# EmaMule/2D-to-3D-Style-Transfer

Measured on AMD Instinct MI355X. Metric: style-transfer iters/sec (512x512, 8 views, cow_mesh), higher is better.
Workload: dtype f32; 1 GPU; BASELINE.json configs[1]: cow_mesh + Style_1, 512x512, 8 views/GPU/iter, texture-only optimisation, white backgrounds (second_approach loop body); texture=512x512, targets_hoisted=content renders + content features + style Grams, parallelism=views sharded dp1, RCCL all-reduce of the texture gradient

## Files before the change

2d-to-3d-style-transfer_amd/csrc/need.hip:

```cpp
#include "common.h"

namespace {

typedef unsigned u32x4 __attribute__((ext_vector_type(4)));

__device__ __forceinline__ void need_segment(const uint8_t *__restrict__ mask, int S, int i, uint8_t *__restrict__ seg) {
    const int segs = S >> 6;
    const int sx = i % segs, y = (i / segs) % S, n = i / (segs * S);
    const uint8_t *m = mask + (size_t)n * S * S;
    unsigned any = 0;
    for (int dy = -1; dy <= 1; ++dy) {
        const int yy = y + dy;
        if (yy < 0 || yy >= S) continue;
        const uint8_t *row = m + (size_t)yy * S + 64 * sx;
        const u32x4 *q = reinterpret_cast<const u32x4 *>(row);
#pragma unroll
        for (int k = 0; k < 4; ++k) {
            const u32x4 v = q[k];
            any |= v[0] | v[1] | v[2] | v[3];
        }
        if (sx > 0) any |= row[-1];
        if (sx + 1 < segs) any |= row[64];
    }
    seg[i] = any ? 1 : 0;
}

__global__ __launch_bounds__(256) void need_segments_kernel(const uint8_t *__restrict__ mask, int S, int total,
                                                            uint8_t *__restrict__ seg) {
    const int i = blockIdx.x * 256 + threadIdx.x;
    if (i < total) need_segment(mask, S, i, seg);
}

struct NeedGeo {
    int tiles_x, tiles_y, rows, cols;
};

__device__ __forceinline__ unsigned seg_block_any(const uint8_t *__restrict__ seg, int S, int n, int ya, int yb, int sa, int sb) {
    const int segs = S >> 6;
    unsigned any = 0;
    for (int y = ya; y <= yb; ++y) {
        const uint8_t *row = seg + ((size_t)n * S + y) * segs;
#pragma unroll 4
        for (int s = sa; s <= sb; ++s) any |= row[s];
    }
    return any;
}

__global__ __launch_bounds__(64) void need_flags_kernel(const uint8_t *__restrict__ seg, int N, int S, NeedGeo g1, NeedGeo g2,
                                                        int total1, int total2, uint8_t *__restrict__ flags) {
    const int i = blockIdx.x * 64 + threadIdx.x;
    if (i >= total1 + total2) return;
    const bool second = i >= total1;
    const NeedGeo g = second ? g2 : g1;
    const int t = second ? i - total1 : i;
    const int per_img = g.tiles_x * g.tiles_y;
    const int n = t / per_img, r = t - n * per_img;
    const int ty = r / g.tiles_x, tx = r - ty * g.tiles_x;
    int ta = ty, tb = ty, ua = tx, ub = tx;
    if (second) {
        const int y0 = 2 * ty * g2.rows, y1 = y0 + 2 * g2.rows - 1;
        const int x0 = 2 * tx * g2.cols, x1 = x0 + 2 * g2.cols - 1;
        ta = max(0, (y0 - 1) / g1.rows); tb = min(g1.tiles_y - 1, (y1 + 1) / g1.rows);
        ua = max(0, (x0 - 1) / g1.cols); ub = min(g1.tiles_x - 1, (x1 + 1) / g1.cols);
    }
    flags[i] = seg_block_any(seg, S, n, ta * g1.rows, tb * g1.rows + g1.rows - 1, (ua * g1.cols) >> 6,
                             (ub * g1.cols + g1.cols - 1) >> 6) ? 1 : 0;
}

__global__ __launch_bounds__(1024) void need_lists_kernel(const uint8_t *__restrict__ flags, int total1, int total2,
                                                          int *__restrict__ list1, int *__restrict__ list2,
                                                          int *__restrict__ counts) {
    __shared__ int scan[1024];
    const int level = blockIdx.x, tid = threadIdx.x;
    const uint8_t *__restrict__ f = level == 0 ? flags : flags + total1;
    int *__restrict__ list = level == 0 ? list1 : list2;
    const int total = level == 0 ? total1 : total2;
    const int per = (total + 1023) / 1024;
    const int lo = min(total, tid * per), hi = min(total, lo + per);
    int cnt = 0;
    for (int t = lo; t < hi; ++t) cnt += f[t];
    scan[tid] = cnt;
    __syncthreads();
    for (int d = 1; d < 1024; d <<= 1) {
        const int v = tid >= d ? scan[tid - d] : 0;
        __syncthreads();
        scan[tid] += v;
        __syncthreads();
    }
    int o = scan[tid] - cnt;
    for (int t = lo; t < hi; ++t)
        if (f[t]) list[o++] = t;
    if (tid == 1023) counts[level] = scan[1023];
}

constexpr int kLists = ST3D_NEED_MAX_LISTS;
constexpr int kListShift[kLists] = {0, 1, 1, 2, 2, 2};
constexpr int kListUnpools[kLists] = {1, 0, 1, 0, 0, 0};

struct BlockLevels {
    int nlists;
    int first;
    int bw[kLists];
    int trows[kLists], tcols[kLists];
    int unpools[kLists];
    int N;
    int total[kLists + 1];
    int *list[kLists];
    int gram_runs;
    int *gram_list, *gram_count;
};

typedef unsigned long long u64;

__device__ __forceinline__ int row_words(int bw) { return (bw + 63) >> 6; }
__device__ __forceinline__ u64 row_tail_mask(int bw, int j) {
    const int left = bw - 64 * j;
    return left >= 64 ? ~0ull : (1ull << left) - 1ull;
}

__global__ __launch_bounds__(256) void need_front_kernel(const uint8_t *__restrict__ mask, int S, int seg_total, int seg_wgs,
                                                         uint8_t *__restrict__ seg, int b0_words, u64 *__restrict__ b0) {
    if ((int)blockIdx.x < seg_wgs) {
        const int i = blockIdx.x * 256 + threadIdx.x;
        if (i < seg_total) need_segment(mask, S, i, seg);
        return;
    }
    const int word = (blockIdx.x - seg_wgs) * 4 + (threadIdx.x >> 6), lane = threadIdx.x & 63;
    if (word >= b0_words) return;
    const int bw = S >> 2, W = row_words(bw);
    const int j = word % W, by = (word / W) % bw, n = word / (W * bw);
    const int bx = 64 * j + lane;
    unsigned any = 0;
    if (bx < bw) {
        const uint8_t *m = mask + (size_t)n * S * S + 4 * bx;
        const int left = bx > 0 ? -1 : 0, right = bx + 1 < bw ? 4 : 3;
#pragma unroll
        for (int r = -1; r <= 4; ++r) {
            const uint8_t *row = m + (size_t)min(max(4 * by + r, 0), S - 1) * S;
            any |= *reinterpret_cast<const unsigned *>(row) | row[left] | row[right];
        }
    }
    const u64 bits = __ballot(any != 0);
    if (lane == 0) b0[word] = bits;
}

__global__ __launch_bounds__(256) void kept_front_kernel(const uint8_t *__restrict__ cover, int S, int k0_words, u64 *__restrict__ k0) {
    const int word = blockIdx.x * 4 + (threadIdx.x >> 6), lane = threadIdx.x & 63;
    if (word >= k0_words) return;
    const int bw = S >> 2, W = row_words(bw);
    const int j = word % W, by = (word / W) % bw, n = word / (W * bw);
    const int bx = 64 * j + lane;
    unsigned any = 0;
    if (bx < bw) {
        const uint8_t *m = cover + (size_t)n * S * S + 4 * bx;
        const int l2 = bx > 0 ? -2 : 0, l1 = bx > 0 ? -1 : 0, r1 = bx + 1 < bw ? 4 : 3, r2 = bx + 1 < bw ? 5 : 3;
#pragma unroll
        for (int r = -2; r <= 5; ++r) {
            const uint8_t *row = m + (size_t)min(max(4 * by + r, 0), S - 1) * S;
            any |= *reinterpret_cast<const unsigned *>(row) | row[l2] | row[l1] | row[r1] | row[r2];
        }
    }
    const u64 bits = __ballot(any != 0);
    if (lane == 0) k0[word] = bits;
}

__device__ __forceinline__ u64 even_bits(u64 x) {
    x &= 0x5555555555555555ull;
    x = (x | (x >> 1)) & 0x3333333333333333ull;
    x = (x | (x >> 2)) & 0x0f0f0f0f0f0f0f0full;
    x = (x | (x >> 4)) & 0x00ff00ff00ff00ffull;
    x = (x | (x >> 8)) & 0x0000ffff0000ffffull;
    x = (x | (x >> 16)) & 0x00000000ffffffffull;
    return x;
}

template <int ROWS>
__device__ __forceinline__ u64 rows_or(const u64 *__restrict__ m, int bw, int W, int ra, int j) {
    const int jc = min(max(j, 0), W - 1);
    u64 v = 0;
#pragma unroll
    for (int d = 0; d < ROWS; ++d) {
        const int r = ra + d;
        const u64 x = m[min(max(r, 0), bw - 1) * W + jc];
        v |= (r >= 0 && r < bw) ? x : 0ull;
    }
    return (j >= 0 && j < W) ? v : 0ull;
}

__device__ __forceinline__ bool cols_any(const u64 *__restrict__ row, int xa, int xb) {
    const int j = xa >> 6, sh = xa & 63, n = xb - xa + 1;
// ... 149 lines not shown
        }
        int o = listed + before + incl - cnt;
        for (int i = 0; lo + i < hi; ++i)
            if (mask >> i & 1u) list[o++] = n0 * per_img + lo + i;
        listed += all;
        __syncthreads();
    }
    if (tid == 0) (gram ? L.gram_count : counts + k)[0] = (!gram && tc == 4) ? listed / 4 : listed;
}

bool blocks_fit(int S) {
    if (S <= 0 || (S % 64) != 0) return false;
    const size_t bw = (size_t)S / 4;
    return bw * ((bw + 63) / 64) <= (size_t)kMaxMapWords;
}

int geo_of(int H, int W, NeedGeo *g) {
    int rows = 0, cols = 0;
    if (!st3d_wino43_tile_geometry(H, W, &rows, &cols)) return 0;
    *g = NeedGeo{W / cols, H / rows, rows, cols};
    return 1;
}

}

extern "C" int st3d_need_levels(int S) {
    NeedGeo g;
    if (S <= 0 || (S % 64) != 0) return 0;
    if (!geo_of(S, S, &g)) return 1;
    if (!geo_of(S / 2, S / 2, &g)) return 2;
    return 3;
}

extern "C" size_t st3d_need_workspace_bytes(int N, int S) {
    NeedGeo g1, g2;
    size_t b = 0;
    if (N <= 0 || st3d_need_levels(S) < 2) return 0;
    geo_of(S, S, &g1);
    b = (size_t)N * g1.tiles_x * g1.tiles_y;
    if (geo_of(S / 2, S / 2, &g2)) b += (size_t)N * g2.tiles_x * g2.tiles_y;
    return b;
}

extern "C" int st3d_need_build(const uint8_t *mask, int N, int S, int levels, uint8_t *seg, void *workspace, size_t workspace_bytes,
                               int *list1, int *list2, int *counts, st3d_stream_t stream) {
    ST3D_CHECK_ARG(mask && seg && N > 0);
    ST3D_CHECK_ARG(levels >= 1 && levels <= st3d_need_levels(S));
    ST3D_CHECK_ARG(((uintptr_t)mask & 15) == 0);
    ST3D_CHECK_ARG((long)N * S * S < (1L << 31));
    ST3D_CHECK_ARG(levels < 2 || (list1 && counts && workspace && workspace_bytes >= st3d_need_workspace_bytes(N, S)));
    ST3D_CHECK_ARG(levels < 3 || list2);
    hipStream_t s = st3d::as_stream(stream);
    const int total = N * S * (S / 64);
    need_segments_kernel<<<st3d::cdiv(total, 256), 256, 0, s>>>(mask, S, total, seg);
    ST3D_LAUNCH_CHECK();
    if (levels >= 2) {
        NeedGeo g1, g2;
        geo_of(S, S, &g1);
        g2 = g1;
        if (levels >= 3) geo_of(S / 2, S / 2, &g2);
        const int total1 = N * g1.tiles_x * g1.tiles_y, total2 = levels >= 3 ? N * g2.tiles_x * g2.tiles_y : 0;
        uint8_t *flags = reinterpret_cast<uint8_t *>(workspace);
        need_flags_kernel<<<st3d::cdiv(total1 + total2, 64), 64, 0, s>>>(seg, N, S, g1, g2, total1, total2, flags);
        ST3D_LAUNCH_CHECK();
        need_lists_kernel<<<levels - 1, 1024, 0, s>>>(flags, total1, total2, list1, list2, counts);
        ST3D_LAUNCH_CHECK();
    }
    return ST3D_OK;
}

extern "C" int st3d_need_blocks_lists(int S) {
    if (!blocks_fit(S)) return 0;
    int k = 0;
    while (k < kLists && st3d_wino43_tile_geometry(S >> kListShift[k], S >> kListShift[k], nullptr, nullptr)) ++k;
    return k;
}

extern "C" size_t st3d_need_blocks_tiles(int N, int S, int k) {
    if (N <= 0 || k < 0 || k >= st3d_need_blocks_lists(S)) return 0;
    const size_t bw = (size_t)(S >> kListShift[k]) / 4;
    return (size_t)N * bw * bw / 16;
}

extern "C" size_t st3d_need_blocks_entries(int N, int S, int k, int tile_cols) {
    return st3d_need_blocks_tiles(N, S, k) * (tile_cols == 16 ? 4 : 1);
}

extern "C" size_t st3d_need_blocks_gram_runs(int N, int S) {
    const int R = S / 2;
    if (N <= 0 || st3d_need_blocks_lists(S) < 2 || (R % 64) != 0) return 0;
    return (size_t)N * R * (R / 64);
}

static size_t b0_words(int N, int S) {
    const size_t bw = (size_t)S / 4;
    return (size_t)N * bw * ((bw + 63) / 64);
}

extern "C" size_t st3d_need_blocks_workspace_bytes(int N, int S) {
    if (N <= 0 || st3d_need_blocks_lists(S) == 0) return 0;
    return b0_words(N, S) * sizeof(u64);
}

static int fill_levels(BlockLevels *Lp, int N, int S, int first, int nlists, const int *tile_cols, int *const *lists) {
    BlockLevels &L = *Lp;
    memset(&L, 0, sizeof(L));
    L.nlists = nlists;
    L.first = first;
    L.N = N;
    for (int k = 0; k < nlists; ++k) {
        const int R = S >> kListShift[k];
        int rows = 0, cols = 0;
        st3d_wino43_tile_geometry(R, R, &rows, &cols);
        if (tile_cols && tile_cols[k]) cols = tile_cols[k];
        ST3D_CHECK_ARG(k < first || lists[k]);
        ST3D_CHECK_ARG((cols == 64 && R % 64 == 0) || (cols == 32 && R % 32 == 0) || cols == 16);
        ST3D_CHECK_ARG(k < first || cols != 16 || ((uintptr_t)lists[k] & 15) == 0);
        L.bw[k] = R / 4;
        L.trows[k] = cols == 32 ? 2 : 1;
        L.tcols[k] = cols / 4;
        L.unpools[k] = kListUnpools[k];
        L.total[k] = (int)st3d_need_blocks_tiles(N, S, k);
        L.list[k] = k < first ? nullptr : lists[k];
    }
    return ST3D_OK;
}

extern "C" int st3d_need_blocks_build(const uint8_t *mask, int N, int S, int nlists, const int *tile_cols, uint8_t *seg,
                                      void *workspace, size_t workspace_bytes, int *const *lists, int *counts, int *gram_list,
                                      int *gram_count, st3d_stream_t stream) {
    ST3D_CHECK_ARG(mask && seg && N > 0);
    ST3D_CHECK_ARG(!gram_list || (gram_count && nlists >= 2 && st3d_need_blocks_gram_runs(N, S) > 0));
    ST3D_CHECK_ARG(nlists >= 1 && nlists <= st3d_need_blocks_lists(S));
    ST3D_CHECK_ARG(((uintptr_t)mask & 15) == 0);
    ST3D_CHECK_ARG((long)N * S * S < (1L << 31));
    ST3D_CHECK_ARG(lists && counts && workspace && workspace_bytes >= st3d_need_blocks_workspace_bytes(N, S));
    ST3D_CHECK_ARG(((uintptr_t)workspace & 15) == 0);
    BlockLevels L;
    ST3D_TRY(fill_levels(&L, N, S, 0, nlists, tile_cols, lists));
    if (gram_list) {
        L.gram_runs = (int)(st3d_need_blocks_gram_runs(N, S) / N);
        L.gram_list = gram_list;
        L.gram_count = gram_count;
    }
    L.total[nlists] = N * L.gram_runs;
    hipStream_t s = st3d::as_stream(stream);
    const int words = (int)b0_words(N, S);
    const int total = N * S * (S / 64), seg_wgs = st3d::cdiv(total, 256);
    u64 *bits = reinterpret_cast<u64 *>(workspace);
    need_front_kernel<<<seg_wgs + st3d::cdiv(words, 4), 256, 0, s>>>(mask, S, total, seg_wgs, seg, words, bits);
    ST3D_LAUNCH_CHECK();
    need_block_lists_kernel<<<nlists + (gram_list ? 1 : 0), 1024, 0, s>>>(bits, L, counts);
    ST3D_LAUNCH_CHECK();
    return ST3D_OK;
}

extern "C" int st3d_kept_build(const uint8_t *cover, int N, int S, int first, int nlists, const int *tile_cols, void *workspace,
                               size_t workspace_bytes, int *const *lists, int *counts, st3d_stream_t stream) {
    ST3D_CHECK_ARG(cover && N > 0);
    ST3D_CHECK_ARG(first >= 0 && first < nlists && nlists <= st3d_need_blocks_lists(S));
    ST3D_CHECK_ARG(((uintptr_t)cover & 15) == 0);
    ST3D_CHECK_ARG((long)N * S * S < (1L << 31));
    ST3D_CHECK_ARG(lists && counts && workspace && workspace_bytes >= st3d_need_blocks_workspace_bytes(N, S));
    ST3D_CHECK_ARG(((uintptr_t)workspace & 15) == 0);
    BlockLevels L;
    ST3D_TRY(fill_levels(&L, N, S, first, nlists, tile_cols, lists));
    hipStream_t s = st3d::as_stream(stream);
    const int words = (int)b0_words(N, S);
    u64 *bits = reinterpret_cast<u64 *>(workspace);
    kept_front_kernel<<<st3d::cdiv(words, 4), 256, 0, s>>>(cover, S, words, bits);
    ST3D_LAUNCH_CHECK();
    need_block_lists_kernel<<<nlists - first, 1024, 0, s>>>(bits, L, counts);
    ST3D_LAUNCH_CHECK();
    return ST3D_OK;
}
```

2d-to-3d-style-transfer_amd/csrc/plan.hip:

```cpp
#include <stdarg.h>
#include <stdlib.h>

#include <algorithm>
#include <vector>

#include "common.h"
#include "epochs.h"
#include "planlists.h"

namespace st3d {
static thread_local char g_err[512] = "";
void set_error(const char *fmt, ...) {
    va_list ap;
    va_start(ap, fmt);
    vsnprintf(g_err, sizeof(g_err), fmt, ap);
    va_end(ap);
}
}

extern "C" int st3d_version(void) { return 100; }
extern "C" const char *st3d_last_error(void) { return st3d::g_err; }

extern "C" int st3d_device_info(int device, int *cu_count, size_t *hbm_bytes, char *name, int name_len) {
    hipDeviceProp_t p;
// ... 70 lines not shown
    ST3D_CHECK_ARG(vgg && w && b);
    const int s = conv_slot(module_idx);
    ST3D_CHECK_ARG(s >= 0);
    ++vgg->sets;
    ST3D_TRY(st3d_conv3x3_pack(w, kConvCout[s], kConvCin[s], vgg->wf[s], vgg->wd[s], stream));
    if (vgg->uf[s]) ST3D_TRY(st3d_wino_pack(w, kConvCout[s], kConvCin[s], vgg->uf[s], vgg->ud[s], stream));
    if (vgg->u6f[s]) ST3D_TRY(st3d_wino43_pack(w, kConvCout[s], kConvCin[s], vgg->u6f[s], vgg->u6d[s], stream));
    ST3D_HIP(hipMemcpyAsync(vgg->bias[s], b, kConvCout[s] * sizeof(float), hipMemcpyDeviceToDevice, st3d::as_stream(stream)));
    vgg->set[s] = true;
    return ST3D_OK;
}

extern "C" int st3d_vgg_destroy(st3d_vgg *vgg) {
    if (!vgg) return ST3D_OK;
    for (int i = 0; i < 16; ++i) {
        if (vgg->wf[i]) (void)hipFree(vgg->wf[i]);
        if (vgg->wd[i]) (void)hipFree(vgg->wd[i]);
        if (vgg->uf[i]) (void)hipFree(vgg->uf[i]);
        if (vgg->ud[i]) (void)hipFree(vgg->ud[i]);
        if (vgg->u6f[i]) (void)hipFree(vgg->u6f[i]);
        if (vgg->u6d[i]) (void)hipFree(vgg->u6d[i]);
        if (vgg->bias[i]) (void)hipFree(vgg->bias[i]);
    }
    delete vgg;
    return ST3D_OK;
}

struct GraphKey {
    int n = 0, denom = 0;
    bool want_grad = false, masked = false, flat = false;
    float sw = 0.f, cw = 0.f;
    bool guided = false;
    bool operator==(const GraphKey &o) const {
        return n == o.n && denom == o.denom && want_grad == o.want_grad && masked == o.masked && flat == o.flat && sw == o.sw && cw == o.cw &&
               guided == o.guided;
    }
};

struct st3d_plan {
    st3d_vgg *vgg = nullptr;
    int B = 0, S = 0;
    std::vector<void *> owned;
    size_t bytes = 0;
    float *act[kModules] = {};
    int C[kModules] = {}, H[kModules] = {}, W[kModules] = {};
    template <typename T> T *at(T *buf, int m, int i0) const { return buf + (size_t)i0 * C[m] * H[m] * W[m]; }
    uint8_t *pidx[5] = {};
    float *gbuf[2] = {};
    size_t gbuf_floats = 0;
    Route route[16];
    bool fused_tap0 = false;
    float *content_target = nullptr;
    float *style_gram[5] = {};
    int style_batch = 0;
    bool have_content = false, have_style = false;
    float *gram[5] = {}, *D[5] = {};
    float *gram_ws = nullptr;
    size_t gram_ws_bytes = 0;
    float *partials = nullptr;
    int last_n = 0;
    bool prof = false;
    struct Ev { int fam, module; hipEvent_t a, b; };
    std::vector<Ev> evs;
    std::vector<hipEvent_t> pool;
    float fam_ms[ST3D_PROFILE_FAMILIES] = {};
    int fam_n[ST3D_PROFILE_FAMILIES] = {};
    std::vector<int> l_tag;
    std::vector<float> l_ms;
    int use_graph = 0;
    hipGraphExec_t gexec = nullptr;
    hipStream_t cap_stream = nullptr;
    float *g_in = nullptr, *g_grad = nullptr, *g_loss = nullptr, *g_color = nullptr;
    uint8_t *g_mask = nullptr;
    GraphKey gkey;
    bool gwarm = false;
    PlanDecisions d;
    uint8_t *need_flags = nullptr, *flat_ws = nullptr, *keep_ws = nullptr;
    size_t need_flags_bytes = 0, flat_ws_bytes = 0, keep_ws_bytes = 0;
    static constexpr int kEpochSlots = 3;
    struct Lists {
        uint8_t *need_seg = nullptr;
        int *need_list[ST3D_NEED_MAX_LISTS] = {}, *need_cnt = nullptr;
        int *need_gram_list = nullptr, *need_gram_cnt = nullptr;
        int *kept_list[ST3D_NEED_MAX_LISTS] = {}, *kept_cnt = nullptr;
        int *flat_list[3] = {}, *flat_map[3] = {}, *flat_cnt = nullptr;
    };
    struct ListSet {
        Lists whole;
        Lists grp[2];
        uint8_t *c1_skip = nullptr;
        bool have_need = false, have_flat = false;
        bool have_kept = false;
        bool have_grp_fwd = false, have_grp_need = false;
    };
    ListSet sets[1 + kEpochSlots];
    ListSet *ls = &sets[0];
    st3d::EpochSlots<kEpochSlots> epochs;
    st3d::CleanRecord clean;
    bool conv1_skip = false;
    bool flat_check = false;
    hipStream_t gstream = nullptr;
    hipEvent_t ev_fork[2] = {}, ev_join[2] = {};
    int split_calls[2] = {};
    int guide_n = 0;
    float *guide_q = nullptr, *guide_w0 = nullptr, *guide_sums = nullptr, *guide_parts = nullptr;
    const float *guide_plane(int level) const {
        size_t off = 0;
        for (int l = 0; l < level; ++l) off += (size_t)guide_n * (S >> l) * (S >> l);
        return guide_q + off;
    }
};

namespace {

template <typename T>
int dev_alloc(st3d_plan *p, T **ptr, size_t count) {
    const size_t bytes = count * sizeof(T);
    if (hipMalloc(reinterpret_cast<void **>(ptr), bytes) != hipSuccess) {
        st3d::set_error("st3d_plan_create: hipMalloc(%zu bytes) failed", bytes);
        return ST3D_E_NOMEM;
    }
    p->owned.push_back(*ptr);
    p->bytes += bytes;
    static const bool poison = [] { const char *e = getenv("ST3D_POISON_PLAN"); return e && e[0] == '1'; }();
    if (poison) (void)hipMemset(*ptr, 0xFF, bytes);
    return ST3D_OK;
}

struct Scope {
    st3d_plan *p; int fam, module; hipStream_t s; hipEvent_t a, b; bool on;
    Scope(st3d_plan *p_, int fam_, hipStream_t s_, int module_ = 99) : p(p_), fam(fam_), module(module_), s(s_), on(p_->prof) {
        if (!on) return;
        auto get = [&]() {
            hipEvent_t e;
            if (!p->pool.empty()) { e = p->pool.back(); p->pool.pop_back(); } else { (void)hipEventCreate(&e); }
            return e;
        };
        a = get(); b = get();
        (void)hipEventRecord(a, s);
    }
    ~Scope() {
        if (!on) return;
        (void)hipEventRecord(b, s);
        p->evs.push_back({fam, module, a, b});
    }
};

enum { F_CONV_FWD = 0, F_CONV_DGRAD = 1, F_POOL = 2, F_GRAM_FWD = 3, F_GRAM_BWD = 4, F_ELEM = 5, F_CONVX_FWD = 6, F_CONVX_DGRAD = 7,
       F_CONV43_FWD = 8, F_CONV43_DGRAD = 9,
       F_CONV43_DGRAD_NEED = 10, F_CONVX_DGRAD_NEED = 11, F_GRAM_BWD_NEED = 12,
       F_CONV43_FWD_FLAT = 13, F_FLAT_FILL = 14,
       F_CONVX_FWD_FLAT = 15 };
static_assert(F_CONVX_FWD_FLAT + 1 == ST3D_PROFILE_FAMILIES, "profile families");

struct Keyed {
    uint64_t epoch;
    const uint8_t *cover;
    const float *rgb;
    int flat_done;
    int kept_done;
    bool clean_call = false;
};
struct FwdLists {
    const st3d_plan::Lists &lists;
    const uint8_t *c1_skip;
    const bool *kept_on;
};

bool split_ok(const st3d_plan *p, int dir, int n, bool keyed) {
    return keyed && (p->d.split_mode & dir) && p->gstream && !p->prof && !p->use_graph && p->guide_n == 0 && n >= 4 && n % 2 == 0;
}
int split_join(st3d_plan *p, int dir, hipStream_t s) {
    ST3D_HIP(hipEventRecord(p->ev_join[dir], p->gstream));
    ST3D_HIP(hipStreamWaitEvent(s, p->ev_join[dir], 0));
    return ST3D_OK;
}
template <typename Fn>
int run_split(st3d_plan *p, int dir, hipStream_t s, Fn fn) {
    ST3D_HIP(hipEventRecord(p->ev_fork[dir], s));
    ST3D_HIP(hipStreamWaitEvent(p->gstream, p->ev_fork[dir], 0));
    int rc = ST3D_OK;
    for (int g = 0; g < 2 && rc == ST3D_OK; ++g) rc = fn(g, g == 0 ? s : p->gstream);
    const int rj = split_join(p, dir, s);
    if (rc != ST3D_OK || rj != ST3D_OK) return rc != ST3D_OK ? rc : rj;
    ++p->split_calls[dir];
    return ST3D_OK;
}

int build_forward_lists(st3d_plan *p, st3d_plan::Lists &L, const uint8_t *cover, int images, int flat, bool want_flat, uint8_t *c1_skip,
                        bool want_kept, hipStream_t s) {
    if (want_flat) {
        Scope sc(p, F_ELEM, s);
        ST3D_TRY(st3d_flat_build_cover(cover, images, p->S, flat, p->flat_ws, p->flat_ws_bytes, L.flat_list[0], L.flat_map[0], L.flat_list[1],
                                       L.flat_map[1], L.flat_list[2], L.flat_map[2], L.flat_cnt, s));
        if (c1_skip) ST3D_TRY(st3d_conv1_skip_build(cover, images, p->S, p->S, c1_skip, s));
    }
    if (want_kept) {
        Scope sc(p, F_ELEM, s);
        ST3D_TRY(st3d_kept_build(cover, images, p->S, p->d.keep_first, kKeepFirst + p->d.keep_levels, p->d.keep_cols, p->keep_ws,
                                 p->keep_ws_bytes, L.kept_list, L.kept_cnt, s));
    }
    return ST3D_OK;
}

int build_need_lists(st3d_plan *p, st3d_plan::Lists &L, const uint8_t *mask, int images, int need, bool gram, hipStream_t s) {
    Scope sc(p, F_ELEM, s);
    if (p->d.need_blocks && need >= 2)
        return st3d_need_blocks_build(mask, images, p->S, need - 1, p->d.need_cols, L.need_seg, p->need_flags, p->need_flags_bytes, L.need_list,
                                      L.need_cnt, gram ? L.need_gram_list : nullptr, L.need_gram_cnt, s);
    return st3d_need_build(mask, images, p->S, need, L.need_seg, p->need_flags, p->need_flags_bytes, L.need_list[0], L.need_list[1], L.need_cnt, s);
}

int kept_launch(st3d_plan *p, int cs, const float *x, float *y, float *yp, uint8_t *yi, int n, int cols, const st3d_plan::Lists &L,
                hipStream_t s) {
    const st3d_vgg *v = p->vgg;
    const int m = kConvIdx[cs], k = cs - 1, Cin = kConvCin[cs], Cout = kConvCout[cs], H = p->H[m], W = p->W[m];
    Scope sc(p, F_CONV43_FWD_FLAT, s, m);
    if (cols == 16) return st3d_wino43_fwd_strips(x, v->u6f[cs], v->bias[cs], y, n, Cin, Cout, H, W, 1, L.kept_list[k], L.kept_cnt + k, s);
    return st3d_wino43_fwd_tiles_geo(x, v->u6f[cs], v->bias[cs], y, yp, yi, n, Cin, Cout, H, W, 1, cols, L.kept_list[k], L.kept_cnt + k, s);
}

int forward_chain(st3d_plan *p, const float *x, int i0, int n, int upto, bool keep_full, hipStream_t s, int flat, int keep, bool fill,
                  const FwdLists &fl) {
    const st3d_vgg *v = p->vgg;
    const st3d_plan::Lists &L = fl.lists;
    auto act = [&](int m) { return p->at(p->act[m], m, i0); };
    auto on = [&](int k) { return !fl.kept_on || fl.kept_on[k]; };
    for (int m = 0; m <= upto; ++m) {
        const int cs = conv_slot(m), ps = pool_slot(m);
        if (cs >= 0) {
            if (!v->set[cs]) {
                st3d::set_error("st3d_plan_forward: weights of module %d were never set", m);
                return ST3D_E_STATE;
            }
            const int Cin = kConvCin[cs], Cout = kConvCout[cs], H = p->H[m], W = p->W[m];
            const uint8_t route = p->route[cs].fwd;
            if (route == DIRECT && cs == 0 && !fill && fl.c1_skip) {
                Scope sc(p, F_CONVX_FWD_FLAT, s, m);
                ST3D_TRY(st3d_conv3x3_fwd_skip(x, v->wf[cs], v->bias[cs], act(m), n, Cin, Cout, H, W, 1, fl.c1_skip, s));
                x = act(m);
                continue;
            }
            if (route == DIRECT) {
                Scope sc(p, F_CONVX_FWD, s, m);
                ST3D_TRY(st3d_conv3x3_fwd(x, v->wf[cs], v->bias[cs], act(m), n, Cin, Cout, H, W, 1, s));
                x = act(m);
                continue;
            }
            const int pool_m = m + 2;
            const int pps = (pool_m <= upto) ? pool_slot(pool_m) : -1;
            float *yfull = (pps < 0 || keep_full) ? act(m) : nullptr;
            float *yp = pps >= 0 ? act(pool_m) : nullptr;
            uint8_t *yi = pps >= 0 ? p->at(p->pidx[pps], pool_m, i0) : nullptr;
            const bool listed = cs >= 1 && (cs <= flat || (cs > kKeepFirst && cs <= kKeepFirst + keep));
            const int kept_cols = !(listed && !fill && keep > 0 && on(cs - 1)) ? 0 : cs <= flat ? p->d.shallow_cols[cs - 1] : p->d.keep_cols[cs - 1];
            if (kept_cols) {
                ST3D_TRY(kept_launch(p, cs, x, yfull, yp, yi, n, kept_cols, L, s));
            } else if (cs >= 1 && cs <= flat) {
                {
                    Scope sc(p, F_CONV43_FWD_FLAT, s, m);
                    ST3D_TRY(st3d_wino43_fwd_tiles(x, v->u6f[cs], v->bias[cs], yfull, yp, yi, n, Cin, Cout, H, W, 1, L.flat_list[cs - 1],
                                                   L.flat_cnt + (cs - 1), s));
                }
                if (fill) {
                    Scope sc(p, F_FLAT_FILL, s, m);
                    ST3D_TRY(st3d_flat_fill(L.flat_map[cs - 1], yfull, yp, yi, n, Cout, H, W, s));
                }
            } else if (route == WINO43) {
                Scope sc(p, F_CONV43_FWD, s, m);
                ST3D_TRY(st3d_wino43_fwd(x, v->u6f[cs], v->bias[cs], yfull, yp, yi, n, Cin, Cout, H, W, 1, s));
            } else {
                Scope sc(p, F_CONV_FWD, s, m);
                ST3D_TRY(st3d_wino_fwd(x, v->uf[cs], v->bias[cs], yfull, yp, yi, n, Cin, Cout, H, W, 1, s));
            }
            x = pps >= 0 ? yp : act(m);
            if (pps >= 0) m = pool_m;
        } else if (ps >= 0) {
            Scope sc(p, F_POOL, s, m);
            ST3D_TRY(st3d_maxpool2x2_fwd(x, act(m), p->at(p->pidx[ps], m, i0), n, p->C[m], p->H[m - 1], p->W[m - 1], s));
            x = act(m);
        }
    }
    return ST3D_OK;
}

int forward(st3d_plan *p, const float *imgs, int n, int upto, bool keep_full, hipStream_t s, const float *flat_color = nullptr,
            Keyed *key = nullptr) {
    const st3d_vgg *v = p->vgg;
    st3d_plan::ListSet *ls = p->ls;
    int flat = 0;
    if (flat_color)
        while (flat < p->d.flat_levels && kConvIdx[flat + 1] <= upto) ++flat;
    int keep = 0;
    if (key && flat == p->d.flat_levels)
        while (keep < p->d.keep_levels && kConvIdx[kKeepFirst + 1 + keep] <= upto) ++keep;
    const bool fill = !(key && flat > 0 && p->clean.matches(key->epoch, n, flat, key->rgb, v->sets, keep));
    p->clean.clear();
    if (flat > 0 && !key) {
        Scope sc(p, F_ELEM, s);
        st3d_plan::Lists &L = ls->whole;
        ST3D_TRY(st3d_flat_build(imgs, flat_color, n, p->S, flat, p->flat_ws, p->flat_ws_bytes, L.flat_list[0], L.flat_map[0], L.flat_list[1],
                                 L.flat_map[1], L.flat_list[2], L.flat_map[2], L.flat_cnt, s));
    } else if (flat > 0 && p->flat_check) {
        int bad = 0, *cnt = p->sets[0].whole.flat_cnt + 3;
        ST3D_TRY(st3d_flat_check_cover(imgs, flat_color, key->cover, n, p->S, p->flat_ws, p->flat_ws_bytes, cnt, s));
        ST3D_HIP(hipMemcpyAsync(&bad, cnt, sizeof(int), hipMemcpyDeviceToHost, s));
        ST3D_HIP(hipStreamSynchronize(s));
        if (bad) {
            st3d::set_error("st3d_plan_loss_keyed: a pixel outside the coverage differs from the background colour");
            return ST3D_E_STATE;
        }
    }
    if (key) {
        const bool want_flat = flat > 0 && !ls->have_flat, want_kept = !fill && keep > 0 && !ls->have_kept;
        ST3D_TRY(build_forward_lists(p, ls->whole, key->cover, n, flat, want_flat, ls->c1_skip, false, s));
        ls->have_flat |= want_flat;
        key->flat_done = flat; key->kept_done = keep; key->clean_call = !fill;
        ST3D_TRY(build_forward_lists(p, ls->whole, key->cover, n, flat, false, nullptr, want_kept, s));
        ls->have_kept |= want_kept;
    }
    if (!fill && upto == 28 && !keep_full && split_ok(p, SPLIT_FWD, n, key != nullptr)) {
        const int h = n / 2;
        for (int g = 0; g < 2 && !ls->have_grp_fwd; ++g)
            ST3D_TRY(build_forward_lists(p, ls->grp[g], key->cover + (size_t)g * h * p->S * p->S, h, flat, true, nullptr, keep > 0, s));
        ls->have_grp_fwd = true;
        ST3D_TRY(run_split(p, 0, s, [&](int g, hipStream_t gs) {
            const FwdLists fl{ls->grp[g], ls->c1_skip ? ls->c1_skip + st3d_conv1_skip_tiles(1, p->S, p->S) * (size_t)g * h : nullptr,
                              p->d.grp_kept_on};
            return forward_chain(p, imgs + (size_t)g * h * 3 * p->S * p->S, g * h, h, upto, keep_full, gs, flat, keep, fill, fl);
        }));
    } else {
        ST3D_TRY(forward_chain(p, imgs, 0, n, upto, keep_full, s, flat, keep, fill, FwdLists{ls->whole, ls->c1_skip, nullptr}));
    }
    p->last_n = n;
    return ST3D_OK;
}

__global__ __launch_bounds__(256) void square_kernel(const float *__restrict__ q, size_t n, float *__restrict__ w) {
    const size_t stride = (size_t)gridDim.x * blockDim.x;
    for (size_t i = (size_t)blockIdx.x * blockDim.x + threadIdx.x; i < n; i += stride) w[i] = q[i] * q[i];
}

__global__ __launch_bounds__(256) void add_kernel(const float *__restrict__ x, size_t n, int accumulate, float *__restrict__ g) {
    const size_t stride = (size_t)gridDim.x * blockDim.x;
    for (size_t i = (size_t)blockIdx.x * blockDim.x + threadIdx.x; i < n; i += stride) g[i] = accumulate ? g[i] + x[i] : x[i];
}

__global__ __launch_bounds__(256) void unpool_add_kernel(const float *__restrict__ gp, const uint8_t *__restrict__ idx,
                                                         const float *__restrict__ add, size_t planes, int H, int W,
                                                         float *__restrict__ out) {
    const int Hp = H / 2, Wp = W / 2;
    const size_t n = planes * (size_t)Hp * Wp;
    const size_t i = (size_t)blockIdx.x * blockDim.x + threadIdx.x;
    if (i >= n) return;
    const int xo = (int)(i % Wp), yo = (int)((i / Wp) % Hp);
    const size_t pl = i / ((size_t)Wp * Hp);
    const float g = gp ? gp[i] : 0.f;
    const int k = gp ? idx[i] : -1;
    const size_t base = pl * H * W + (size_t)(2 * yo) * W + 2 * xo;
#pragma unroll
    for (int q = 0; q < 4; ++q) {
        const size_t o = base + (size_t)(q >> 1) * W + (q & 1);
        out[o] = (q == k ? g : 0.f) + (add ? add[o] : 0.f);
    }
}

struct DgradOpts {
    bool pregated = false;
    const float *out_gate = nullptr;
    const float *add_target = nullptr;
    float add_coef = 0.f;
    const int *tile_list = nullptr, *n_active = nullptr;
    int tile_cols = 0;
};

int dgrad_step(st3d_plan *p, int cs, const float *g, bool g_is_pooled, int pool_of_g, float *dst, int n, hipStream_t s,
               const DgradOpts &o = {}, int i0 = 0) {
    const st3d_vgg *v = p->vgg;
    const int m = kConvIdx[cs];
    const int Cin = kConvCin[cs], Cout = kConvCout[cs], H = p->H[m], W = p->W[m];
    const bool wino = p->route[cs].dgrad_wino;
    const bool w43 = p->route[cs].dgrad_w43 && o.pregated;
    if (o.tile_list && !w43) {
        st3d::set_error("st3d_plan_loss_masked: the input gradient of module %d is not an F(4x4,3x3) launch", m);
        return ST3D_E_STATE;
    }
    Scope sc(p, o.tile_list ? F_CONV43_DGRAD_NEED : w43 ? F_CONV43_DGRAD : (wino ? F_CONV_DGRAD : F_CONVX_DGRAD), s, m);
    const int pm = g_is_pooled ? kPoolIdx[pool_of_g] : 0;
    const uint8_t *pidx = g_is_pooled ? p->at(p->pidx[pool_of_g], pm, i0) : nullptr;
    const float *pooled = g_is_pooled ? p->at(p->act[pm], pm, i0) : nullptr;
    const float *act_m = p->at(p->act[m], m, i0);
    if (o.tile_list)
        ST3D_TRY(st3d_wino43_dgrad_chain_tiles_geo(g, pidx, v->u6d[cs], o.out_gate, o.add_target, o.add_coef, dst, n, Cin, Cout, H, W,
                                                   o.tile_cols, o.tile_list, o.n_active, s));
    else if (w43)
        ST3D_TRY(st3d_wino43_dgrad_chain(g, pidx, v->u6d[cs], o.out_gate, o.add_target, o.add_coef, dst, n, Cin, Cout, H, W, s));
    else if (wino && (o.pregated || o.out_gate))
        ST3D_TRY(st3d_wino_dgrad_chain(g, (g_is_pooled || o.pregated) ? nullptr : act_m, pidx, o.pregated ? nullptr : pooled,
                                       v->ud[cs], o.out_gate, o.add_target, o.add_coef, dst, n, Cin, Cout, H, W, s));
    else if (g_is_pooled && wino)
        ST3D_TRY(st3d_wino_dgrad_unpool(g, pidx, pooled, v->ud[cs], dst, n, Cin, Cout, H, W, s));
    else if (g_is_pooled)
        ST3D_TRY(st3d_conv3x3_dgrad_unpool(g, pidx, pooled, v->wd[cs], dst, n, Cin, Cout, H, W, s));
    else if (wino)
        ST3D_TRY(st3d_wino_dgrad(g, act_m, v->ud[cs], dst, n, Cin, Cout, H, W, s));
    else
        ST3D_TRY(st3d_conv3x3_dgrad(g, act_m, v->wd[cs], dst, n, Cin, Cout, H, W, s));
    return ST3D_OK;
}

}

extern "C" int st3d_plan_create(st3d_plan **out, st3d_vgg *vgg, int B, int S) {
    ST3D_CHECK_ARG(out && vgg);
    ST3D_CHECK_ARG(B > 0 && S >= 16);
// ... 25 lines not shown
        Route &r = p->route[cs];
        if (v->uf[cs] && st3d_wino_supported(Cin, Cout, H, W)) r.fwd = w43(Cin, Cout) ? WINO43 : WINO;
        r.dgrad_wino = v->ud[cs] && st3d_wino_supported(Cout, Cin, H, W);
        r.dgrad_w43 = r.dgrad_wino && w43(Cout, Cin);
        r.gate_taps = v->pregate && r.dgrad_wino && (Cout % 32) == 0;
        r.gate_dst = v->pregate && cs > 0 && r.dgrad_wino && p->route[cs - 1].dgrad_wino;
    }
    p->fused_tap0 = v->fuse_tap0 && st3d_conv1_bwd_supported(S, S) && gmax >= (size_t)B * 27 * S * S;
    PlanFacts f;
    f.B = B; f.S = S;
    int dev = 0;
    if (hipGetDevice(&dev) != hipSuccess || hipDeviceGetAttribute(&f.cus, hipDeviceAttributeMultiprocessorCount, dev) != hipSuccess || f.cus <= 0) f.cus = 256;
    for (int cs = 0; cs < 16; ++cs) { f.H[cs] = p->H[kConvIdx[cs]]; f.route[cs] = p->route[cs]; }
    f.fused_tap0 = p->fused_tap0;
    f.need_levels = st3d_need_levels(S);
    f.blocks_lists = st3d_need_blocks_lists(S);
    f.flat_levels = st3d_flat_levels(S);
    for (int k = 0; k < ST3D_NEED_MAX_LISTS; ++k) st3d_wino43_tile_geometry(f.H[k + 1], f.H[k + 1], &f.geo_rows[k], &f.geo_cols[k]);
    f.gram_segs = st3d_gram_bwd_segs_supported(p->C[kConvIdx[2]], f.H[2] * f.H[2]) != 0;
    f.gram_runs = st3d_need_blocks_gram_runs(B, S);
    p->d = decide_lists(f, [](const char *name) -> const char * { return getenv(name); });
    const PlanDecisions &d = p->d;
    for (int i = 0; i < 2; ++i) alloc(&p->gbuf[i], gmax);
    alloc(&p->content_target, (size_t)B * p->C[kContentTap] * p->H[kContentTap] * p->W[kContentTap]);
    for (int i = 0; i < 5; ++i) {
        const int m = kStyleTap[i];
        const size_t cc = (size_t)B * p->C[m] * p->C[m];
        alloc(&p->style_gram[i], cc);
        alloc(&p->gram[i], cc);
        alloc(&p->D[i], cc);
    }
    for (int n = 1; n <= B; ++n) {
        st3d_gram_item items[5];
        for (int i = 0; i < 5; ++i) items[i] = st3d_gram_item{nullptr, nullptr, n, p->C[kStyleTap[i]], p->H[kStyleTap[i]] * p->W[kStyleTap[i]]};
        const size_t ws = st3d_gram_multi_workspace_bytes(items, 5);
        if (ws > wsmax) wsmax = ws;
    }
    p->gram_ws_bytes = wsmax;
    alloc(&p->gram_ws, wsmax / sizeof(float));
    alloc(&p->partials, (size_t)8 * st3d_reduce_partials());
    alloc(&p->g_in, (size_t)B * 3 * S * S);
    alloc(&p->g_grad, (size_t)B * 3 * S * S);
    alloc(&p->g_loss, (size_t)4);
    if (d.need_levels >= 1) {
        alloc(&p->g_mask, (size_t)B * S * S);
        p->need_flags_bytes = d.need_blocks ? st3d_need_blocks_workspace_bytes(B, S) : st3d_need_workspace_bytes(B, S);
        if (d.need_levels >= 2) alloc(&p->need_flags, p->need_flags_bytes);
    }
    if (d.flat_levels >= 1) {
        p->flat_ws_bytes = st3d_flat_workspace_bytes(B, S);
        alloc(&p->flat_ws, p->flat_ws_bytes);
        alloc(&p->g_color, (size_t)4);
    }
    if (d.keep_levels >= 1) {
        p->keep_ws_bytes = st3d_need_blocks_workspace_bytes(B, S);
        alloc(&p->keep_ws, p->keep_ws_bytes);
    }
    auto alloc_lists = [&](st3d_plan::Lists &L, int images, bool need, bool kept) {
        if (need) {
            alloc(&L.need_seg, (size_t)images * S * (S / 64));
            alloc(&L.need_cnt, (size_t)ST3D_NEED_MAX_LISTS);
            if (d.need_gram) {
                alloc(&L.need_gram_list, st3d_need_blocks_gram_runs(images, S));
                alloc(&L.need_gram_cnt, (size_t)1);
            }
            for (int l = 0; l + 2 <= d.need_levels; ++l) {
                if (d.need_blocks) {
                    alloc(&L.need_list[l], st3d_need_blocks_entries(images, S, l, d.need_cols[l]));
                    continue;
                }
                int rows = 0, cols = 0;
                st3d_wino43_tile_geometry(S >> l, S >> l, &rows, &cols);
                alloc(&L.need_list[l], (size_t)images * ((S >> l) / rows) * ((S >> l) / cols));
            }
        }
        if (d.flat_levels >= 1) {
            alloc(&L.flat_cnt, (size_t)4);
            for (int k = 0; k < d.flat_levels; ++k) {
                alloc(&L.flat_list[k], (size_t)st3d_flat_tiles(images, S, k));
                alloc(&L.flat_map[k], (size_t)st3d_flat_tiles(images, S, k));
            }
        }
        if (kept) {
            alloc(&L.kept_cnt, (size_t)ST3D_NEED_MAX_LISTS);
            for (int k = d.keep_first; k < kKeepFirst + d.keep_levels; ++k)
                alloc(&L.kept_list[k], st3d_need_blocks_entries(images, S, k, d.keep_cols[k]));
        }
    };
    if (d.split_mode && rc == ST3D_OK) {
        bool ok = hipStreamCreateWithFlags(&p->gstream, hipStreamNonBlocking) == hipSuccess;
        for (int dir = 0; dir < 2; ++dir)
            ok = ok && hipEventCreateWithFlags(&p->ev_fork[dir], hipEventDisableTiming) == hipSuccess &&
                 hipEventCreateWithFlags(&p->ev_join[dir], hipEventDisableTiming) == hipSuccess;
        if (!ok) { st3d::set_error("st3d_plan_create: the split batch's stream and events could not be made"); rc = ST3D_E_HIP; }
    }
    auto flag = [](const char *name, bool dflt) { const char *e = getenv(name); return e && e[0] ? e[0] != '0' : dflt; };
    p->flat_check = flag("ST3D_FLAT_CHECK", false);
    p->conv1_skip = d.flat_levels >= 1 && p->route[0].fwd == DIRECT && flag("ST3D_FLAT_CONV1", true);
    for (int i = 0; i <= st3d_plan::kEpochSlots; ++i) {
        st3d_plan::ListSet &ls = p->sets[i];
        alloc_lists(ls.whole, B, d.need_levels >= 1, i >= 1 && d.keep_levels >= 1);
        if (i == 0) continue;
        if (d.split_mode)
            for (st3d_plan::Lists &G : ls.grp) alloc_lists(G, B / 2, d.need_levels >= 1 && d.need_blocks, d.keep_levels >= 1);
        if (p->conv1_skip) alloc(&ls.c1_skip, st3d_conv1_skip_tiles(B, S, S));
    }
    if (rc != ST3D_OK) { st3d_plan_destroy(p); return rc; }
    *out = p;
    return ST3D_OK;
}

extern "C" int st3d_plan_destroy(st3d_plan *p) {
    if (!p) return ST3D_OK;
    for (void *b : p->owned) (void)hipFree(b);
    if (p->gexec) (void)hipGraphExecDestroy(p->gexec);
    if (p->cap_stream) (void)hipStreamDestroy(p->cap_stream);
    if (p->gstream) (void)hipStreamDestroy(p->gstream);
    for (int d = 0; d < 2; ++d) {
        if (p->ev_fork[d]) (void)hipEventDestroy(p->ev_fork[d]);
        if (p->ev_join[d]) (void)hipEventDestroy(p->ev_join[d]);
    }
    for (auto &e : p->evs) { (void)hipEventDestroy(e.a); (void)hipEventDestroy(e.b); }
    for (auto &e : p->pool) (void)hipEventDestroy(e);
    delete p;
    return ST3D_OK;
}

extern "C" size_t st3d_plan_bytes(const st3d_plan *p) { return p ? p->bytes : 0; }

extern "C" int st3d_plan_forward(st3d_plan *p, const float *imgs, int n, int upto_module, st3d_stream_t stream) {
    ST3D_CHECK_ARG(p && imgs);
    ST3D_CHECK_ARG(n > 0 && n <= p->B && upto_module >= 0 && upto_module < kModules);
    st3d::TraceRange tr("vgg_forward");
    return forward(p, imgs, n, upto_module, true, st3d::as_stream(stream));
}

extern "C" int st3d_plan_activation(st3d_plan *p, int module_idx, float **ptr, int *C, int *H, int *W) {
    ST3D_CHECK_ARG(p && ptr && module_idx >= 0 && module_idx < kModules);
    *ptr = p->act[module_idx];
    if (C) *C = p->C[module_idx];
    if (H) *H = p->H[module_idx];
    if (W) *W = p->W[module_idx];
    return ST3D_OK;
}

extern "C" int st3d_plan_set_content(st3d_plan *p, const float *content, int n, st3d_stream_t stream) {
    ST3D_CHECK_ARG(p && content && n > 0 && n <= p->B);
    hipStream_t s = st3d::as_stream(stream);
    ST3D_TRY(forward(p, content, n, kContentTap, false, s));
    const size_t cnt = (size_t)n * p->C[kContentTap] * p->H[kContentTap] * p->W[kContentTap];
    ST3D_HIP(hipMemcpyAsync(p->content_target, p->act[kContentTap], cnt * sizeof(float), hipMemcpyDeviceToDevice, s));
    p->have_content = true;
    return ST3D_OK;
}

extern "C" int st3d_plan_get_content_features(st3d_plan *p, float *out, int n, st3d_stream_t stream) {
    ST3D_CHECK_ARG(p && out && n > 0 && n <= p->B);
    if (!p->have_content) {
        st3d::set_error("st3d_plan_get_content_features: no content target set");
        return ST3D_E_STATE;
    }
    const size_t cnt = (size_t)n * p->C[kContentTap] * p->H[kContentTap] * p->W[kContentTap];
    ST3D_HIP(hipMemcpyAsync(out, p->content_target, cnt * sizeof(float), hipMemcpyDeviceToDevice, st3d::as_stream(stream)));
    return ST3D_OK;
}

extern "C" int st3d_plan_set_content_features(st3d_plan *p, const float *feat, int n, st3d_stream_t stream) {
    ST3D_CHECK_ARG(p && feat && n > 0 && n <= p->B);
    const size_t cnt = (size_t)n * p->C[kContentTap] * p->H[kContentTap] * p->W[kContentTap];
    ST3D_HIP(hipMemcpyAsync(p->content_target, feat, cnt * sizeof(float), hipMemcpyDeviceToDevice, st3d::as_stream(stream)));
    p->have_content = true;
    return ST3D_OK;
}

static int grams_of_taps(st3d_plan *p, int n, float *const *out, hipStream_t s, bool guided = false) {
    st3d_gram_item items[5];
    const float *q[5];
    for (int i = 0; i < 5; ++i) {
        const int m = kStyleTap[i];
        items[i] = st3d_gram_item{p->act[m], out[i], n, p->C[m], p->H[m] * p->W[m]};
        q[i] = guided ? p->guide_plane(i) : nullptr;
    }
    if (guided) return st3d_gram_fwd_multi_weighted(items, q, 5, p->gram_ws, p->gram_ws_bytes, s);
    return st3d_gram_fwd_multi(items, 5, p->gram_ws, p->gram_ws_bytes, s);
}

extern "C" int st3d_plan_set_style_guidance(st3d_plan *p, const float *mask, int n, st3d_stream_t stream) {
    ST3D_CHECK_ARG(p);
    if (!mask) { p->guide_n = 0; return ST3D_OK; }
    ST3D_CHECK_ARG(n > 0 && n <= p->B);
    hipStream_t s = st3d::as_stream(stream);
    p->guide_n = 0;
    if (!p->guide_q) ST3D_TRY(dev_alloc(p, &p->guide_q, st3d_guidance_floats(p->B, p->S)));
    if (!p->guide_w0) ST3D_TRY(dev_alloc(p, &p->guide_w0, (size_t)p->B * p->S * p->S));
    if (!p->guide_sums) ST3D_TRY(dev_alloc(p, &p->guide_sums, (size_t)5 * p->B));
    if (!p->guide_parts) ST3D_TRY(dev_alloc(p, &p->guide_parts, st3d_guidance_partials(p->B, p->S)));
    ST3D_TRY(st3d_guidance_build(mask, n, p->S, p->guide_q, p->guide_sums, p->guide_parts, s));
    const size_t cnt = (size_t)n * p->S * p->S;
    square_kernel<<<(unsigned)std::min<size_t>((cnt + 255) / 256, 65535), 256, 0, s>>>(p->guide_q, cnt, p->guide_w0);
    ST3D_LAUNCH_CHECK();
    p->guide_n = n;
    return ST3D_OK;
}

extern "C" int st3d_plan_set_style(st3d_plan *p, const float *style, int style_batch, int n, st3d_stream_t stream) {
    ST3D_CHECK_ARG(p && style && n > 0 && n <= p->B && (style_batch == 1 || style_batch == n));
    hipStream_t s = st3d::as_stream(stream);
    ST3D_TRY(forward(p, style, style_batch, 28, false, s));
    {
        Scope sc(p, F_GRAM_FWD, s);
        ST3D_TRY(grams_of_taps(p, style_batch, p->style_gram, s));
    }
    if (p->style_batch != style_batch && p->gexec) {
        (void)hipGraphExecDestroy(p->gexec); p->gexec = nullptr; p->gwarm = false;
    }
    p->style_batch = style_batch;
    p->have_style = true;
    return ST3D_OK;
}

static int plan_loss_enqueue(st3d_plan *p, const float *current, int n, int batch_denom, float style_weight,
                             float content_weight, float *loss_out, float *grad_current, const uint8_t *need_mask, const float *flat_color, hipStream_t s,
// ... 417 lines not shown
```

2d-to-3d-style-transfer_amd/csrc/planlists.h:

```cpp
#pragma once
#include <stdint.h>
#include <stdlib.h>
#include <string.h>

#include <algorithm>

#include "../../include/st3d.h"

namespace st3d {

constexpr int kModules = 37;
constexpr int kConvIdx[16] = {0, 2, 5, 7, 10, 12, 14, 16, 19, 21, 23, 25, 28, 30, 32, 34};
constexpr int kConvCin[16] = {3, 64, 64, 128, 128, 256, 256, 256, 256, 512, 512, 512, 512, 512, 512, 512};
constexpr int kConvCout[16] = {64, 64, 128, 128, 256, 256, 256, 256, 512, 512, 512, 512, 512, 512, 512, 512};
constexpr int kPoolIdx[5] = {4, 9, 18, 27, 36};

inline int conv_slot(int module_idx) {
    for (int i = 0; i < 16; ++i)
        if (kConvIdx[i] == module_idx) return i;
    return -1;
}
inline int pool_slot(int module_idx) {
    for (int i = 0; i < 5; ++i)
        if (kPoolIdx[i] == module_idx) return i;
    return -1;
}

enum : uint8_t { DIRECT, WINO, WINO43 };
struct Route {
    uint8_t fwd = DIRECT;
    bool dgrad_wino = false;
    bool dgrad_w43 = false;
    bool gate_taps = false;
    bool gate_dst = false;
};

#define ST3D_SPLIT_BATCH_DEFAULT 1
enum { SPLIT_FWD = 1, SPLIT_BWD = 2 };
constexpr int kKeepFirst = 3, kKeepMax = 3;

struct PlanFacts {
    int B = 0, S = 0, cus = 0;
    int H[16] = {};
    Route route[16];
    bool fused_tap0 = false;
    int need_levels = 0, blocks_lists = 0, flat_levels = 0;
    int geo_rows[ST3D_NEED_MAX_LISTS] = {}, geo_cols[ST3D_NEED_MAX_LISTS] = {};
    bool gram_segs = false;
    size_t gram_runs = 0;
};

struct PlanDecisions {
    int need_levels = 0;
    bool need_blocks = false;
    int need_cols[ST3D_NEED_MAX_LISTS] = {};
    bool need_gram = false;
    int flat_levels = 0;
    int keep_levels = 0;
    int keep_cols[ST3D_NEED_MAX_LISTS] = {};
    int shallow_cols[3] = {};
    int keep_first = kKeepFirst;
    int split_mode = 0;
    bool grp_kept_on[ST3D_NEED_MAX_LISTS] = {};
    int grp_need_levels = 0;
    bool grp_need_gram = false;
};

inline int next_cols(const char *&cur, int dflt, bool last_repeats) {
    if (!cur || (last_repeats && !cur[0])) return dflt;
    const int v = atoi(cur);
    if (const char *c = strchr(cur, ',')) cur = c + 1;
    else if (!last_repeats) cur = "";
    return v;
}

inline PlanDecisions decide_lists(const PlanFacts &f, const char *(*env)(const char *)) {
    PlanDecisions d;
    const int B = f.B, hb = f.B / 2;
    const Route *route = f.route;
    auto flag = [&](const char *name, bool dflt) { const char *e = env(name); return e && e[0] ? e[0] != '0' : dflt; };
    auto capped = [&](int levels, const char *name) {
        const char *e = env(name);
        return (e && atoi(e) >= 0 && atoi(e) < levels) ? atoi(e) : levels;
    };
    const bool need_force = flag("ST3D_NEED_FORCE", false), keep_force = flag("ST3D_KEEP_FORCE", false);
    auto two_rounds = [&](int images, int R, int channels) {
        return (long)images * (R / 4) * (R / 4) / 16 >= 2L * (f.cus / std::max(1, channels / 64));
    };
    auto gram_rounds = [&](int images) { return (long)images * (f.H[2] * f.H[2] / 64) >= 2L * 4 * f.cus; };
    auto fits = [](int cols, int R, bool strips_ok) {
        return (cols == 64 && R % 64 == 0) || (cols == 32 && R % 32 == 0 && R % 8 == 0) || (cols == 16 && strips_ok);
    };
    auto pools = [](int cs) { return pool_slot(kConvIdx[cs] + 2) >= 0; };

    int need_ok = f.fused_tap0 ? 1 : 0;
    if (need_ok == 1 && route[2].gate_dst && route[1].dgrad_w43) need_ok = 2;
    if (need_ok == 2 && route[2].dgrad_w43) need_ok = 3;
    int need_max = f.need_levels;
    d.need_blocks = need_ok >= 2 && f.blocks_lists >= 2 && flag("ST3D_NEED_BLOCKS", true);
    if (d.need_blocks) {
        need_max = 1 + f.blocks_lists;
        for (int cs = 3; cs <= ST3D_NEED_MAX_LISTS && need_ok == cs; ++cs)
            if (route[cs].dgrad_w43 && (cs == 4 ? route[cs].gate_taps : route[cs + 1].gate_dst) &&
                (need_force || two_rounds(B, f.H[cs], kConvCin[cs])))
                need_ok = cs + 1;
        static const int kDefaultCols[ST3D_NEED_MAX_LISTS] = {16, 16, 16, 32, 16, 16};
        const char *tile = env("ST3D_NEED_TILE");
        for (int k = 0; k < ST3D_NEED_MAX_LISTS; ++k) {
            const int R = f.H[k + 1], cols = next_cols(tile, kDefaultCols[k], true);
            const bool on = fits(cols, R, f.geo_rows[k] != 0) && cols != f.geo_cols[k] && (need_force || two_rounds(B, R, kConvCin[k + 1]));
            d.need_cols[k] = on ? cols : 0;
        }
    }
    d.need_levels = capped(std::min(need_ok, need_max), "ST3D_NEED_DEPTH");
    d.need_gram = d.need_blocks && d.need_levels >= 3 && flag("ST3D_NEED_GRAM", true) && route[2].gate_taps && f.gram_segs &&
                  f.gram_runs > 0 && (need_force || gram_rounds(B));

    int flat_ok = 0;
    while (flat_ok < 3 && route[flat_ok + 1].fwd == WINO43) ++flat_ok;
    d.flat_levels = capped(std::min(flat_ok, f.flat_levels), "ST3D_FLAT_DEPTH");

    int keep_ok = 0;
    const char *tile = env("ST3D_KEEP_TILE");
    while (d.flat_levels == 3 && keep_ok < kKeepMax) {
        const int k = kKeepFirst + keep_ok, cs = k + 1, R = f.H[cs];
        if (k >= f.blocks_lists || route[cs].fwd != WINO43 || pools(cs)) break;
        if (!keep_force && !two_rounds(B, R, kConvCout[cs])) break;
        int cols = next_cols(tile, 16, true);
        if (cols == 0) cols = f.geo_cols[k];
        if (!fits(cols, R, true)) break;
        d.keep_cols[k] = cols;
        ++keep_ok;
    }
    d.keep_levels = capped(keep_ok, "ST3D_KEEP_DEPTH");
    static const int kDefaultShallow[3] = {32, 16, 32};
    const char *sh = env("ST3D_KEEP_SHALLOW");
    for (int k = 0; k < 3 && d.keep_levels >= 1; ++k) {
        const int cs = k + 1, R = f.H[cs], cols = next_cols(sh, kDefaultShallow[k], false);
        if (!fits(cols, R, !pools(cs)) || (!keep_force && !two_rounds(B, R, kConvCout[cs]))) continue;
        d.shallow_cols[k] = cols;
        if (k < d.keep_first) d.keep_first = k;
    }
    for (int k = d.keep_first; k < 3; ++k) d.keep_cols[k] = d.shallow_cols[k] ? d.shallow_cols[k] : 16;

    const char *sb = env("ST3D_SPLIT_BATCH");
    if (sb && sb[0]) d.split_mode = strcmp(sb, "fwd") == 0 ? SPLIT_FWD : strcmp(sb, "bwd") == 0 ? SPLIT_BWD : sb[0] == '1' ? (SPLIT_FWD | SPLIT_BWD) : 0;
    else d.split_mode = ST3D_SPLIT_BATCH_DEFAULT;
    if (B < 4 || d.flat_levels < 1) d.split_mode = 0;
    for (int k = 0; k < ST3D_NEED_MAX_LISTS; ++k) {
        const bool walked = k < 3 ? d.shallow_cols[k] != 0 : k - kKeepFirst < d.keep_levels;
        d.grp_kept_on[k] = walked && (keep_force || two_rounds(hb, f.H[k + 1], kConvCout[k + 1]));
    }
    d.grp_need_levels = d.need_levels;
    for (int cs = 3; cs <= ST3D_NEED_MAX_LISTS && cs + 1 <= d.grp_need_levels; ++cs)
        if (!need_force && !two_rounds(hb, f.H[cs], kConvCin[cs])) d.grp_need_levels = cs;
    d.grp_need_gram = d.need_gram && (need_force || gram_rounds(hb));
    return d;
}

}
```

2d-to-3d-style-transfer_amd/csrc/wino43.hip:

```cpp
#include <stdlib.h>
#include <string.h>

#include <type_traits>

#include "common.h"

namespace {

typedef float f32x4 __attribute__((ext_vector_type(4)));
typedef float f32x2 __attribute__((ext_vector_type(2)));
typedef unsigned u32x4 __attribute__((ext_vector_type(4)));
typedef unsigned u32x2 __attribute__((ext_vector_type(2)));
typedef int i32x4 __attribute__((ext_vector_type(4)));

constexpr int KS6 = 16;
constexpr int NK6 = KS6 / 4;
constexpr int EX6 = 6 * 32 * 16 * 2 * 2;
template <int TC>
struct Geo43 {
    static constexpr int TR = 16 / TC;
    static constexpr int ROWS = 4 * TR, COLS = 4 * TC;
    static constexpr int XLEFT = TC == 4 ? 2 : 4;
    static constexpr int LOFF0 = 5 - XLEFT;
    static constexpr int PAIRS = TC == 4 ? 2 * TC + 2 : 2 * TC + 4;
    static constexpr int PITCH = TC == 4 ? 4 * TC + 8 : 4 * TC + 12;
    static constexpr int CHS = TR * 6 * PITCH;
    static constexpr int TSTAGE = KS6 * CHS;
    static constexpr int HALF_ITEMS = KS6 * TR * PAIRS;
    static constexpr int SMEM = 3 * TSTAGE + EX6;
    static_assert(HALF_ITEMS <= 768 && SMEM * 4 <= 160 * 1024, "tile geometry does not fit the workgroup");
};
constexpr int NT6 = 768;

struct Wino43Args {
    const float *x;
    const uint8_t *idx;
    const float *U;
    const float *bias;
    float *y;
    float *yp;
    uint8_t *yidx;
    int N, Cin, Cout, H, W, relu, tiles_x, tiles_y, n_ct;
    const float *gate;
    const float *addt;
    float addc;
    int xpc;
    unsigned magic_x, magic_y;
    const int *tile_list;
    const int *n_active;
};

template <typename T>
__device__ __forceinline__ void bt6(T d0, T d1, T d2, T d3, T d4, T d5, T &t0, T &t1, T &t2, T &t3, T &t4, T &t5) {
    const T p = d4 - 4.f * d2, q = d3 - 4.f * d1;
    t1 = p + q; t2 = p - q;
    t0 = 4.f * d0 + (d4 - 5.f * d2);
    const T r = d4 - d2, s = 2.f * (d3 - d1);
    t3 = r + s; t4 = r - s;
    t5 = 4.f * d1 + (d5 - 5.f * d3);
}

#if defined(ST3D_W43_DIAG) && ST3D_W43_DIAG == 5
#define W43_GATE_VO(v) (a.N >= 0 ? kOob : (v))
#else
#define W43_GATE_VO(v) (v)
#endif

template <int MODE, int EPI, int GATE, int BH, int TC, bool LIST, bool STRIPS>
__device__ __forceinline__ void wino43_body(const Wino43Args &a, float *smem) {
    using G = Geo43<TC>;
    static_assert(!STRIPS || (LIST && EPI == 0 && G::TR == 4), "strips come from a list and leave through the plain epilogue");
    constexpr int SROWS = STRIPS ? 4 : G::ROWS;
    const int tid = threadIdx.x;
    const int lane = tid & 63, wave = __builtin_amdgcn_readfirstlane(tid >> 6);
    const int wa = wave >> 1;
    constexpr int bh = BH;
    const int tx = lane & 15, kq = lane >> 4;

    const int ct = blockIdx.x % a.n_ct, nslots = gridDim.x / a.n_ct;
    int slot = blockIdx.x / a.n_ct;
    if (a.xpc > 1) slot = (slot % a.xpc) * (nslots / a.xpc) + slot / a.xpc;
    const int npix = LIST ? __builtin_amdgcn_readfirstlane(a.n_active[0]) : a.tiles_x * a.tiles_y * a.N;
    const int co0 = ct * 64;
    int n = 0, x0 = 0, y0 = 0;
    auto decode = [&](int pix, int &tn, int &ty0, int &tx0) __attribute__((always_inline)) {
        const int r2 = a.tiles_x == 1 ? pix : (int)__umulhi((unsigned)pix, a.magic_x);
        const int txi = pix - r2 * a.tiles_x;
        tn = a.tiles_y == 1 ? r2 : (int)__umulhi((unsigned)r2, a.magic_y);
        tx0 = txi * G::COLS; ty0 = (r2 - tn * a.tiles_y) * SROWS;
    };
    auto decode_step = [&](const i32x4 &ent, int &tn, i32x4 &org) __attribute__((always_inline)) {
        tn = 0;
#pragma unroll
        for (int i = 3; i >= 0; --i) {
            int en, ey, ex;
            decode(ent[i] < 0 ? 0 : ent[i], en, ey, ex);
            org[i] = ent[i] < 0 ? -1 : (ey << 16 | ex);
            tn = ent[i] < 0 ? tn : en;
        }
    };
    auto pick = [&](const i32x4 &org, int i) __attribute__((always_inline)) {
        int v = org[0];
#pragma unroll
        for (int j = 1; j < 4; ++j) v = i == j ? org[j] : v;
        return v;
    };
    const int H = a.H, W = a.W;
    const size_t HW = (size_t)H * W;
    const int Hp = H >> 1, Wp = W >> 1;
    constexpr bool UNPOOL = MODE == 3;
    const size_t in_plane = UNPOOL ? (size_t)Hp * Wp : HW;
    const int nstages = a.Cin / KS6;
    const unsigned kOob = 0x80000000u;

    const int s_ci = tid / (G::TR * G::PAIRS), s_rem = tid - s_ci * (G::TR * G::PAIRS);
    const int s_tr = s_rem / G::PAIRS;
    const int s_col = 2 * (s_rem - s_tr * G::PAIRS);
    const bool s_on = tid < G::HALF_ITEMS;
    unsigned voff[6];
    unsigned rowbit[UNPOOL ? 6 : 1];
#pragma unroll
    for (int r = 0; r < 6; ++r)
        if (UNPOOL) rowbit[r] = (unsigned)((r + 1) & 1) << 1;
    const unsigned img_bytes = (unsigned)((size_t)a.Cin * in_plane * 4);
    __amdgpu_buffer_rsrc_t rx, ridx;
    int stile = 0, ctile = 0;
    unsigned nxt = 0;
    auto list_at = [&](int pos) __attribute__((always_inline)) { return pos < npix ? (unsigned)a.tile_list[pos] : 0u; };
    i32x4 sent = {-1, -1, -1, -1}, cent = sent, corg = sent, nxts = sent;
    auto step_at = [&](int pos) __attribute__((always_inline)) {
        return pos < npix ? *reinterpret_cast<const i32x4 *>(a.tile_list + (size_t)pos * 4) : i32x4{-1, -1, -1, -1};
    };
    auto uniform4 = [&](const i32x4 &v) __attribute__((always_inline)) {
        return i32x4{__builtin_amdgcn_readfirstlane(v[0]), __builtin_amdgcn_readfirstlane(v[1]),
                     __builtin_amdgcn_readfirstlane(v[2]), __builtin_amdgcn_readfirstlane(v[3])};
    };
    auto stage_tile = [&](int pix) __attribute__((always_inline)) {
        const bool live = pix < npix;
        if (STRIPS) {
            i32x4 org;
            decode_step(sent, n, org);
            const int mine = pick(org, s_tr);
            const bool on = live && s_on && mine >= 0;
            const int sy0 = mine >> 16, sx0 = mine & 0xffff;
#pragma unroll
            for (int r = 0; r < 6; ++r) {
                const int gy = sy0 - 1 + r, gx0 = sx0 - G::XLEFT + s_col;
                const bool ok = on && gy >= 0 && gy < H && gx0 >= 0 && gx0 < W;
                if (UNPOOL) voff[r] = ok ? (unsigned)((s_ci * in_plane + (size_t)(gy >> 1) * Wp + (gx0 >> 1)) * 4) : kOob;
                else voff[r] = ok ? (unsigned)((s_ci * in_plane + (size_t)gy * W + gx0) * 4) : kOob;
            }
        } else {
        decode(live ? (LIST ? stile : pix) : 0, n, y0, x0);
#pragma unroll
// ... 315 lines not shown
                stage_tile(spix);
            }
            if (sc >= nstages) sc -= nstages;
            stage(c, sc, pb);
            pb = pb == 2 ? 0 : pb + 1;
        }
        int cn, cy0 = 0, cx0 = 0;
        if (STRIPS) decode_step(cent, cn, corg);
        else decode(LIST ? ctile : cpix, cn, cy0, cx0);
#if defined(ST3D_W43_DIAG) && ST3D_W43_DIAG == 2
        if (a.N < 0) { float sacc = 0.f; for (int b = 0; b < 3; ++b) for (int cb = 0; cb < 4; ++cb) for (int r = 0; r < 4; ++r) sacc += acc[b][cb][r]; ex[tid] = sacc; }
        uload(0, u4[0]); uload(1, u4[1]); uload(2, u4[2]);
#else
        epilogue(cn, cy0, cx0);
#endif
        asm volatile("" : "+s"(spix));
        if (STRIPS) {
            cent = sent;
            nxts = step_at(spix + nslots);
        } else if (LIST) {
            ctile = stile;
            nxt = list_at(spix + nslots);
        }
        stage_tile(spix);
#pragma unroll
        for (int b = 0; b < 3; ++b)
#pragma unroll
            for (int cb = 0; cb < 4; ++cb) acc[b][cb] = f32x4{0.f, 0.f, 0.f, 0.f};
    }
}

template <int MODE, int EPI, int GATE, int TC, bool LIST = false, bool STRIPS = false>
__global__ __launch_bounds__(NT6, 3) void wino43_kernel(const Wino43Args a) {
    extern __shared__ __attribute__((aligned(16))) float smem[];
    if (__builtin_amdgcn_readfirstlane(threadIdx.x >> 6) & 1) wino43_body<MODE, EPI, GATE, 1, TC, LIST, STRIPS>(a, smem);
    else wino43_body<MODE, EPI, GATE, 0, TC, LIST, STRIPS>(a, smem);
}

__device__ __forceinline__ size_t upack43_index(int m, int k, int aa, int bb, int K) {
    const int ct = m >> 6, col = m & 63, cb = col >> 4, m16 = col & 15;
    const int kstep = k >> 2, kq = k & 3;
    const int wave = 2 * aa + (bb >= 3 ? 1 : 0), bi = bb % 3;
    const int lane = m16 + 16 * kq;
    return (((((size_t)ct * (K >> 2) + kstep) * 12 + wave) * 3 + bi) * 64 + lane) * 4 + cb;
}

__global__ void wino43_pack_kernel(const float *__restrict__ w, int Cout, int Cin, float *__restrict__ uf, float *__restrict__ ud) {
    const size_t i = (size_t)blockIdx.x * blockDim.x + threadIdx.x;
    if (i >= (size_t)Cout * Cin) return;
    const int co = i / Cin, ci = i % Cin;
    const float *g = w + i * 9;
    const double G[6][3] = {{0.25, 0.0, 0.0}, {-1.0 / 6, -1.0 / 6, -1.0 / 6}, {-1.0 / 6, 1.0 / 6, -1.0 / 6},
                            {1.0 / 24, 1.0 / 12, 1.0 / 6}, {1.0 / 24, -1.0 / 12, 1.0 / 6}, {0.0, 0.0, 1.0}};
    for (int dir = 0; dir < 2; ++dir) {
        float *out = dir == 0 ? uf : ud;
        if (!out) continue;
        double gg[3][3];
        for (int ky = 0; ky < 3; ++ky)
            for (int kx = 0; kx < 3; ++kx) gg[ky][kx] = dir == 0 ? g[ky * 3 + kx] : g[(2 - ky) * 3 + (2 - kx)];
        double t[6][3];
        for (int aa = 0; aa < 6; ++aa)
            for (int kx = 0; kx < 3; ++kx) t[aa][kx] = G[aa][0] * gg[0][kx] + G[aa][1] * gg[1][kx] + G[aa][2] * gg[2][kx];
        for (int aa = 0; aa < 6; ++aa)
            for (int bb = 0; bb < 6; ++bb) {
                const double u = t[aa][0] * G[bb][0] + t[aa][1] * G[bb][1] + t[aa][2] * G[bb][2];
                const size_t o = dir == 0 ? upack43_index(co, ci, aa, bb, Cin) : upack43_index(ci, co, aa, bb, Cout);
                out[o] = (float)u;
            }
    }
}

int tc43(int H, int W) {
    if (H > 0 && W > 0 && (H % 4) == 0 && (W % 64) == 0) return 16;
    if (H > 0 && W > 0 && (H % 8) == 0 && (W % 32) == 0) return 8;
    return 0;
}
bool shape_ok43(int Cin, int Cout, int H, int W) {
    return Cin >= 4 * KS6 && (Cin % 64) == 0 && (Cout % 64) == 0 && tc43(H, W) != 0 &&
           (unsigned long long)Cin * (unsigned long long)H * (unsigned long long)W * 4ull < (1ull << 31) &&
           (unsigned long long)Cout * (unsigned long long)H * (unsigned long long)W * 4ull < (1ull << 31);
}

template <int MODE, int TC>
int launch_wino43_tc(Wino43Args a, hipStream_t s, bool strip_fwd = false) {
    using G = Geo43<TC>;
    constexpr bool kStrips = TC == 4;
    a.tiles_x = a.W / G::COLS;
    a.tiles_y = kStrips ? a.H / 4 : a.H / G::ROWS;
    a.n_ct = a.Cout / 64;
    a.magic_x = (unsigned)((1ull << 32) / (unsigned)a.tiles_x + 1ull);
    a.magic_y = (unsigned)((1ull << 32) / (unsigned)a.tiles_y + 1ull);
    static const int cus = [] {
        int dev = 0, n = 0;
        if (hipGetDevice(&dev) != hipSuccess || hipDeviceGetAttribute(&n, hipDeviceAttributeMultiprocessorCount, dev) != hipSuccess || n <= 0) n = 256;
        return n;
    }();
    const long npix = (long)a.tiles_x * a.tiles_y * a.N / (kStrips ? G::TR : 1);
    long nslots = cus / a.n_ct;
    if (const char *e = getenv("ST3D_W43_SLOTS")) nslots = atol(e);
    if (nslots < 1 || nslots > npix) nslots = npix;
    const long blocks = (long)a.n_ct * nslots;
    a.xpc = 1;
    if (a.n_ct <= 8 && 8 % a.n_ct == 0 && nslots % (8 / a.n_ct) == 0) a.xpc = 8 / a.n_ct;
    if (const char *e = getenv("ST3D_W43_XCD")) { if (atoi(e) == 0) a.xpc = 1; }
    constexpr size_t kSmem = (size_t)G::SMEM * sizeof(float);
    auto go = [&](auto kernel) -> int {
        static const hipError_t attr = hipFuncSetAttribute(reinterpret_cast<const void *>(kernel), hipFuncAttributeMaxDynamicSharedMemorySize, (int)kSmem);
        if (attr != hipSuccess) { st3d::set_error("wino43: hipFuncSetAttribute(MaxDynamicSharedMemorySize): %s", hipGetErrorString(attr)); return ST3D_E_HIP; }
        kernel<<<(unsigned)blocks, NT6, kSmem, s>>>(a);
        ST3D_LAUNCH_CHECK();
        return ST3D_OK;
    };
    if constexpr (kStrips) {
        if (!a.tile_list || !a.n_active) { st3d::set_error("wino43: 16-pixel tile columns come with a strip list and its count"); return ST3D_E_INVALID; }
        if (((uintptr_t)a.tile_list & 15) != 0) { st3d::set_error("wino43: a strip list is 16-byte aligned"); return ST3D_E_INVALID; }
        if (a.yp) { st3d::set_error("wino43: strip lists leave through the plain epilogue, not the fused pool"); return ST3D_E_INVALID; }
        if ((a.bias || a.relu) && !(strip_fwd && MODE == 0 && !a.gate)) { st3d::set_error("wino43: strip lists are for the input-gradient chain"); return ST3D_E_INVALID; }
        if (a.gate && a.addt) {
            if (MODE != 0) { st3d::set_error("wino43: the content-target term rides on ungated input (MODE 0) only"); return ST3D_E_INVALID; }
            return go(wino43_kernel<0, 0, 2, TC, true, true>);
        }
        if (a.gate) return go(wino43_kernel<MODE, 0, 1, TC, true, true>);
        return go(wino43_kernel<MODE, 0, 0, TC, true, true>);
    } else {
    if (a.tile_list) {
        if (!a.n_active) { st3d::set_error("wino43: a tile list without its count"); return ST3D_E_INVALID; }
        if ((a.yp || a.bias || a.relu) && (MODE != 0 || a.gate)) { st3d::set_error("wino43: bias, ReLU and the fused pool belong to the plain forward"); return ST3D_E_INVALID; }
        if (a.yp) return go(wino43_kernel<0, 1, 0, TC, true>);
        if (a.gate && a.addt) {
            if (MODE != 0) { st3d::set_error("wino43: the content-target term rides on ungated input (MODE 0) only"); return ST3D_E_INVALID; }
            return go(wino43_kernel<0, 0, 2, TC, true>);
        }
        if (a.gate) return go(wino43_kernel<MODE, 0, 1, TC, true>);
        return go(wino43_kernel<MODE, 0, 0, TC, true>);
    }
    if (a.yp) {
        if (MODE != 0 || a.gate) { st3d::set_error("wino43: the fused pool belongs to the plain forward"); return ST3D_E_INVALID; }
        return go(wino43_kernel<0, 1, 0, TC>);
    }
    if (a.gate && a.addt) {
        if (MODE != 0) { st3d::set_error("wino43: the content-target term rides on ungated input (MODE 0) only"); return ST3D_E_INVALID; }
        return go(wino43_kernel<0, 0, 2, TC>);
    }
    if (a.gate) return go(wino43_kernel<MODE, 0, 1, TC>);
    return go(wino43_kernel<MODE, 0, 0, TC>);
    }
}

template <int MODE>
int launch_wino43(Wino43Args a, hipStream_t s, int cols = 0, bool strip_fwd = false) {
    const int native = tc43(a.H, a.W);
    if (cols != 0 && !((cols == 64 && native == 16) || (cols == 32 && a.H > 0 && a.W > 0 && (a.H % 8) == 0 && (a.W % 32) == 0) ||
                       (cols == 16 && native != 0))) {
        st3d::set_error("wino43: %d-pixel tile columns do not fit a %d x %d map", cols, a.H, a.W);
        return ST3D_E_INVALID;
    }
    const int tc = cols ? cols / 4 : native;
    if (tc == 4) return launch_wino43_tc<MODE, 4>(a, s, strip_fwd);
    return tc == 16 ? launch_wino43_tc<MODE, 16>(a, s) : launch_wino43_tc<MODE, 8>(a, s);
}

}

extern "C" int st3d_wino43_supported(int Cin, int Cout, int H, int W) { return shape_ok43(Cin, Cout, H, W) ? 1 : 0; }

extern "C" int st3d_wino43_tile_geometry(int H, int W, int *rows, int *cols) {
    const int tc = tc43(H, W);
    if (rows) *rows = tc ? 4 * (16 / tc) : 0;
    if (cols) *cols = 4 * tc;
    return tc != 0;
}

extern "C" size_t st3d_wino43_packed_floats(int Cout, int Cin) { return (size_t)36 * Cout * Cin; }

extern "C" int st3d_wino43_pack(const float *w, int Cout, int Cin, float *u_fwd, float *u_dgrad, st3d_stream_t stream) {
    ST3D_CHECK_ARG(w && (u_fwd || u_dgrad));
    ST3D_CHECK_ARG(Cout > 0 && Cin > 0 && Cout % 64 == 0 && Cin % 64 == 0);
    wino43_pack_kernel<<<st3d::cdiv((long)Cout * Cin, 256), 256, 0, st3d::as_stream(stream)>>>(w, Cout, Cin, u_fwd, u_dgrad);
    ST3D_LAUNCH_CHECK();
    return ST3D_OK;
}

extern "C" int st3d_wino43_fwd(const float *x, const float *u_fwd, const float *bias, float *y, float *y_pooled,
                               uint8_t *pool_idx, int N, int Cin, int Cout, int H, int W, int relu, st3d_stream_t stream) {
    ST3D_CHECK_ARG(x && u_fwd && (y || y_pooled));
    ST3D_CHECK_ARG(N > 0 && shape_ok43(Cin, Cout, H, W));
    ST3D_CHECK_ARG(((uintptr_t)u_fwd & 15) == 0);
    Wino43Args a{x, nullptr, u_fwd, bias, y, y_pooled, pool_idx, N, Cin, Cout, H, W, relu, 0, 0, 0, nullptr, nullptr, 0.f};
    return launch_wino43<0>(a, st3d::as_stream(stream));
}

extern "C" int st3d_wino43_fwd_tiles(const float *x, const float *u_fwd, const float *bias, float *y, float *y_pooled,
                                     uint8_t *pool_idx, int N, int Cin, int Cout, int H, int W, int relu, const int *tile_list,
                                     const int *n_active, st3d_stream_t stream) {
    ST3D_CHECK_ARG(x && u_fwd && (y || y_pooled) && tile_list && n_active);
    ST3D_CHECK_ARG(N > 0 && shape_ok43(Cin, Cout, H, W));
    ST3D_CHECK_ARG(((uintptr_t)u_fwd & 15) == 0);
    Wino43Args a{x, nullptr, u_fwd, bias, y, y_pooled, pool_idx, N, Cin, Cout, H, W, relu, 0, 0, 0, nullptr, nullptr, 0.f};
    a.tile_list = tile_list;
    a.n_active = n_active;
    return launch_wino43<0>(a, st3d::as_stream(stream));
}

extern "C" int st3d_wino43_fwd_tiles_geo(const float *x, const float *u_fwd, const float *bias, float *y, float *y_pooled,
                                         uint8_t *pool_idx, int N, int Cin, int Cout, int H, int W, int relu, int tile_cols,
                                         const int *tile_list, const int *n_active, st3d_stream_t stream) {
    ST3D_CHECK_ARG(x && u_fwd && (y || y_pooled) && tile_list && n_active);
    ST3D_CHECK_ARG(N > 0 && shape_ok43(Cin, Cout, H, W));
    ST3D_CHECK_ARG(((uintptr_t)u_fwd & 15) == 0);
    Wino43Args a{x, nullptr, u_fwd, bias, y, y_pooled, pool_idx, N, Cin, Cout, H, W, relu, 0, 0, 0, nullptr, nullptr, 0.f};
    a.tile_list = tile_list;
    a.n_active = n_active;
    return launch_wino43<0>(a, st3d::as_stream(stream), tile_cols);
}

extern "C" int st3d_wino43_fwd_strips(const float *x, const float *u_fwd, const float *bias, float *y, int N, int Cin, int Cout,
                                      int H, int W, int relu, const int *strip_list, const int *n_steps, st3d_stream_t stream) {
    ST3D_CHECK_ARG(x && u_fwd && y && strip_list && n_steps);
    ST3D_CHECK_ARG(N > 0 && shape_ok43(Cin, Cout, H, W));
    ST3D_CHECK_ARG(((uintptr_t)u_fwd & 15) == 0);
    Wino43Args a{x, nullptr, u_fwd, bias, y, nullptr, nullptr, N, Cin, Cout, H, W, relu, 0, 0, 0, nullptr, nullptr, 0.f};
    a.tile_list = strip_list;
    a.n_active = n_steps;
    return launch_wino43<0>(a, st3d::as_stream(stream), 16, true);
}

extern "C" int st3d_wino43_dgrad_chain(const float *gy, const uint8_t *pool_idx, const float *u_dgrad, const float *out_gate,
                                       const float *add_target, float add_coef, float *gx, int N, int Cin, int Cout, int H,
                                       int W, st3d_stream_t stream) {
    ST3D_CHECK_ARG(gy && u_dgrad && gx);
    ST3D_CHECK_ARG(N > 0 && shape_ok43(Cout, Cin, H, W));
    ST3D_CHECK_ARG(((uintptr_t)u_dgrad & 15) == 0 && ((uintptr_t)out_gate & 15) == 0 && ((uintptr_t)add_target & 15) == 0);
    ST3D_CHECK_ARG(!add_target || out_gate);
    Wino43Args a{gy, pool_idx, u_dgrad, nullptr, gx, nullptr, nullptr, N, Cout, Cin, H, W, 0, 0, 0, 0, out_gate, add_target, add_coef};
    hipStream_t s = st3d::as_stream(stream);
    return pool_idx ? launch_wino43<3>(a, s) : launch_wino43<0>(a, s);
}

extern "C" int st3d_wino43_dgrad_chain_tiles(const float *gy, const uint8_t *pool_idx, const float *u_dgrad, const float *out_gate,
                                             const float *add_target, float add_coef, float *gx, int N, int Cin, int Cout, int H,
                                             int W, const int *tile_list, const int *n_active, st3d_stream_t stream) {
    ST3D_CHECK_ARG(gy && u_dgrad && gx && tile_list && n_active);
    ST3D_CHECK_ARG(N > 0 && shape_ok43(Cout, Cin, H, W));
    ST3D_CHECK_ARG(((uintptr_t)u_dgrad & 15) == 0 && ((uintptr_t)out_gate & 15) == 0 && ((uintptr_t)add_target & 15) == 0);
    ST3D_CHECK_ARG(!add_target || out_gate);
    Wino43Args a{gy, pool_idx, u_dgrad, nullptr, gx, nullptr, nullptr, N, Cout, Cin, H, W, 0, 0, 0, 0, out_gate, add_target, add_coef};
    a.tile_list = tile_list;
    a.n_active = n_active;
    hipStream_t s = st3d::as_stream(stream);
    return pool_idx ? launch_wino43<3>(a, s) : launch_wino43<0>(a, s);
}

extern "C" int st3d_wino43_dgrad_chain_tiles_geo(const float *gy, const uint8_t *pool_idx, const float *u_dgrad, const float *out_gate,
                                                 const float *add_target, float add_coef, float *gx, int N, int Cin, int Cout,
                                                 int H, int W, int tile_cols, const int *tile_list, const int *n_active,
                                                 st3d_stream_t stream) {
    ST3D_CHECK_ARG(gy && u_dgrad && gx && tile_list && n_active);
    ST3D_CHECK_ARG(N > 0 && shape_ok43(Cout, Cin, H, W));
    ST3D_CHECK_ARG(((uintptr_t)u_dgrad & 15) == 0 && ((uintptr_t)out_gate & 15) == 0 && ((uintptr_t)add_target & 15) == 0);
    ST3D_CHECK_ARG(!add_target || out_gate);
    Wino43Args a{gy, pool_idx, u_dgrad, nullptr, gx, nullptr, nullptr, N, Cout, Cin, H, W, 0, 0, 0, 0, out_gate, add_target, add_coef};
    a.tile_list = tile_list;
    a.n_active = n_active;
    hipStream_t s = st3d::as_stream(stream);
    return pool_idx ? launch_wino43<3>(a, s, tile_cols) : launch_wino43<0>(a, s, tile_cols);
}
```

2d-to-3d-style-transfer_amd/st3d/_lib.py:

```python
import ctypes
import os

import torch

_PKG = os.path.dirname(os.path.dirname(os.path.abspath(__file__)))
SO_PATH = os.path.join(_PKG, "lib", "libst3d.so")

c_f32p = ctypes.c_void_p
c_i32p = ctypes.c_void_p
c_u8p = ctypes.c_void_p
c_stream = ctypes.c_void_p
c_int = ctypes.c_int
c_float = ctypes.c_float
c_size = ctypes.c_size_t

SIGNATURES = {
    "st3d_version": (c_int, []),
    "st3d_last_error": (ctypes.c_char_p, []),
    "st3d_device_info": (c_int, [c_int, ctypes.POINTER(c_int), ctypes.POINTER(c_size), ctypes.c_char_p, c_int]),
    "st3d_project_verts": (c_int, [c_f32p, c_int, c_f32p, c_f32p, c_int, c_float, c_f32p, c_stream]),
    "st3d_raster_workspace_bytes": (c_size, [c_int, c_int]),
    "st3d_raster_workspace_bytes_binned": (c_size, [c_int, c_int, c_int]),
    "st3d_raster_fwd": (c_int, [c_f32p, c_i32p, c_int, c_int, c_int, c_int, ctypes.c_void_p, c_size, c_i32p, c_f32p,
                                c_f32p, c_f32p, c_float, c_i32p, c_stream]),
# ... 96 lines not shown
                                  c_f32p, c_f32p, c_stream]),
    "st3d_shade_ss_bwd": (c_int, [c_f32p, c_i32p, c_f32p, c_f32p, c_f32p, c_f32p, c_i32p, c_f32p, c_int, c_int, c_int, c_int,
                                  c_int, c_int, c_f32p, c_f32p, c_f32p, c_stream]),
    "st3d_shade_ss_bwd_det": (c_int, [c_f32p, c_i32p, c_f32p, c_f32p, c_f32p, c_f32p, c_i32p, c_f32p, c_int, c_int, c_int, c_int,
                                      c_int, c_int, c_f32p, c_f32p, c_f32p, ctypes.c_void_p, c_size, c_stream]),
    "st3d_shade_ss_lit_fwd": (c_int, [c_i32p, c_f32p, c_f32p, c_f32p, c_f32p, c_i32p, c_f32p, c_int, c_int, c_int, c_int, c_int,
                                      c_int, c_f32p, c_f32p, c_i32p, c_f32p, c_f32p, c_f32p, c_int, c_int, c_f32p, c_f32p,
                                      c_stream]),
    "st3d_shade_ss_lit_bwd": (c_int, [c_f32p, c_i32p, c_f32p, c_f32p, c_f32p, c_f32p, c_i32p, c_f32p, c_int, c_int, c_int, c_int,
                                      c_int, c_int, c_f32p, c_f32p, c_i32p, c_f32p, c_f32p, c_f32p, c_int, c_int, c_float, c_f32p,
                                      c_f32p, c_f32p, ctypes.c_void_p, c_size, c_stream]),
    "st3d_box_down_fwd": (c_int, [c_f32p, c_int, c_int, c_int, c_int, c_f32p, c_stream]),
    "st3d_box_down_bwd": (c_int, [c_f32p, c_int, c_int, c_int, c_int, c_f32p, c_stream]),
    "st3d_apply_background": (c_int, [c_f32p, c_f32p, c_f32p, c_int, c_int, c_int, c_f32p, c_stream]),
    "st3d_conv3x3_packed_floats": (c_size, [c_int, c_int]),
    "st3d_conv3x3_pack": (c_int, [c_f32p, c_int, c_int, c_f32p, c_f32p, c_stream]),
    "st3d_conv3x3_fwd": (c_int, [c_f32p, c_f32p, c_f32p, c_f32p, c_int, c_int, c_int, c_int, c_int, c_int, c_stream]),
    "st3d_conv1_skip_tiles": (c_size, [c_int, c_int, c_int]),
    "st3d_conv1_skip_build": (c_int, [c_u8p, c_int, c_int, c_int, c_u8p, c_stream]),
    "st3d_conv3x3_fwd_skip": (c_int, [c_f32p, c_f32p, c_f32p, c_f32p, c_int, c_int, c_int, c_int, c_int, c_int, c_u8p, c_stream]),
    "st3d_conv3x3_dgrad": (c_int, [c_f32p, c_f32p, c_f32p, c_f32p, c_int, c_int, c_int, c_int, c_int, c_stream]),
    "st3d_conv3x3_dgrad_unpool": (c_int, [c_f32p, c_u8p, c_f32p, c_f32p, c_f32p, c_int, c_int, c_int, c_int, c_int,
                                          c_stream]),
    "st3d_conv1_bwd_supported": (c_int, [c_int, c_int]),
    "st3d_conv1_bwd_workspace_bytes": (c_size, [c_int, c_int, c_int]),
    "st3d_conv1_bwd": (c_int, [c_f32p, c_f32p, c_f32p, c_float, c_f32p, ctypes.c_void_p, c_size, c_f32p, c_int, c_int, c_int,
                               c_stream]),
    "st3d_conv1_bwd_masked": (c_int, [c_f32p, c_f32p, c_f32p, c_float, c_f32p, ctypes.c_void_p, c_size, c_f32p, c_int, c_int, c_int,
                                      c_u8p, c_u8p, c_stream]),
    "st3d_conv1_bwd_weighted": (c_int, [c_f32p, c_f32p, c_f32p, c_float, c_f32p, ctypes.c_void_p, c_size, c_f32p, c_int, c_int, c_int,
                                        c_f32p, c_u8p, c_u8p, c_stream]),
    "st3d_wino_supported": (c_int, [c_int, c_int, c_int, c_int]),
    "st3d_wino_packed_floats": (c_size, [c_int, c_int]),
    "st3d_wino_pack": (c_int, [c_f32p, c_int, c_int, c_f32p, c_f32p, c_stream]),
    "st3d_wino_fwd": (c_int, [c_f32p, c_f32p, c_f32p, c_f32p, c_f32p, c_u8p, c_int, c_int, c_int, c_int, c_int, c_int,
                              c_stream]),
    "st3d_wino_dgrad": (c_int, [c_f32p, c_f32p, c_f32p, c_f32p, c_int, c_int, c_int, c_int, c_int, c_stream]),
    "st3d_wino_dgrad_unpool": (c_int, [c_f32p, c_u8p, c_f32p, c_f32p, c_f32p, c_int, c_int, c_int, c_int, c_int,
                                       c_stream]),
    "st3d_wino_dgrad_chain": (c_int, [c_f32p, c_f32p, c_u8p, c_f32p, c_f32p, c_f32p, c_f32p, c_float, c_f32p, c_int, c_int, c_int,
                                      c_int, c_int, c_stream]),
    "st3d_wino43_supported": (c_int, [c_int, c_int, c_int, c_int]),
    "st3d_wino43_packed_floats": (c_size, [c_int, c_int]),
    "st3d_wino43_pack": (c_int, [c_f32p, c_int, c_int, c_f32p, c_f32p, c_stream]),
    "st3d_wino43_fwd": (c_int, [c_f32p, c_f32p, c_f32p, c_f32p, c_f32p, c_u8p, c_int, c_int, c_int, c_int, c_int, c_int,
                                c_stream]),
    "st3d_wino43_dgrad_chain": (c_int, [c_f32p, c_u8p, c_f32p, c_f32p, c_f32p, c_float, c_f32p, c_int, c_int, c_int, c_int,
                                        c_int, c_stream]),
    "st3d_wino43_tile_geometry": (c_int, [c_int, c_int, ctypes.POINTER(c_int), ctypes.POINTER(c_int)]),
    "st3d_wino43_dgrad_chain_tiles": (c_int, [c_f32p, c_u8p, c_f32p, c_f32p, c_f32p, c_float, c_f32p, c_int, c_int, c_int, c_int,
                                              c_int, c_i32p, c_i32p, c_stream]),
    "st3d_wino43_fwd_tiles": (c_int, [c_f32p, c_f32p, c_f32p, c_f32p, c_f32p, c_u8p, c_int, c_int, c_int, c_int, c_int, c_int,
                                      c_i32p, c_i32p, c_stream]),
    "st3d_flat_levels": (c_int, [c_int]),
    "st3d_flat_tiles": (c_int, [c_int, c_int, c_int]),
    "st3d_flat_workspace_bytes": (c_size, [c_int, c_int]),
    "st3d_flat_build": (c_int, [c_f32p, c_f32p, c_int, c_int, c_int, ctypes.c_void_p, c_size, c_i32p, c_i32p, c_i32p, c_i32p,
                                c_i32p, c_i32p, c_i32p, c_stream]),
    "st3d_flat_fill": (c_int, [c_i32p, c_f32p, c_f32p, c_u8p, c_int, c_int, c_int, c_int, c_stream]),
    "st3d_flat_build_cover": (c_int, [c_u8p, c_int, c_int, c_int, ctypes.c_void_p, c_size, c_i32p, c_i32p, c_i32p, c_i32p, c_i32p,
                                      c_i32p, c_i32p, c_stream]),
    "st3d_flat_check_cover": (c_int, [c_f32p, c_f32p, c_u8p, c_int, c_int, ctypes.c_void_p, c_size, c_i32p, c_stream]),
    "st3d_need_levels": (c_int, [c_int]),
    "st3d_need_workspace_bytes": (c_size, [c_int, c_int]),
    "st3d_need_build": (c_int, [c_u8p, c_int, c_int, c_int, c_u8p, ctypes.c_void_p, c_size, c_i32p, c_i32p, c_i32p, c_stream]),
    "st3d_need_blocks_lists": (c_int, [c_int]),
    "st3d_need_blocks_tiles": (c_size, [c_int, c_int, c_int]),
    "st3d_need_blocks_entries": (c_size, [c_int, c_int, c_int, c_int]),
    "st3d_need_blocks_workspace_bytes": (c_size, [c_int, c_int]),
    "st3d_need_blocks_build": (c_int, [c_u8p, c_int, c_int, c_int, ctypes.POINTER(c_int), c_u8p, ctypes.c_void_p, c_size,
                                       ctypes.POINTER(ctypes.c_void_p), c_i32p, c_i32p, c_i32p, c_stream]),
    "st3d_need_blocks_gram_runs": (c_size, [c_int, c_int]),
    "st3d_gram_bwd_segs_supported": (c_int, [c_int, c_int]),
    "st3d_gram_bwd_gated_segs": (c_int, [c_f32p, c_f32p, c_f32p, c_int, c_int, c_int, c_float, c_int, c_i32p, c_i32p, c_f32p,
                                         c_stream]),
    "st3d_wino43_dgrad_chain_tiles_geo": (c_int, [c_f32p, c_u8p, c_f32p, c_f32p, c_f32p, c_float, c_f32p, c_int, c_int, c_int,
                                                  c_int, c_int, c_int, c_i32p, c_i32p, c_stream]),
    "st3d_wino43_fwd_tiles_geo": (c_int, [c_f32p, c_f32p, c_f32p, c_f32p, c_f32p, c_u8p, c_int, c_int, c_int, c_int, c_int, c_int,
                                          c_int, c_i32p, c_i32p, c_stream]),
    "st3d_wino43_fwd_strips": (c_int, [c_f32p, c_f32p, c_f32p, c_f32p, c_int, c_int, c_int, c_int, c_int, c_int, c_i32p, c_i32p,
                                       c_stream]),
    "st3d_kept_build": (c_int, [c_u8p, c_int, c_int, c_int, c_int, ctypes.POINTER(c_int), ctypes.c_void_p, c_size,
                                ctypes.POINTER(ctypes.c_void_p), c_i32p, c_stream]),
    "st3d_maxpool2x2_fwd": (c_int, [c_f32p, c_f32p, c_u8p, c_int, c_int, c_int, c_int, c_stream]),
    "st3d_gram_workspace_bytes": (c_size, [c_int, c_int, c_int]),
    "st3d_gram_fwd": (c_int, [c_f32p, c_int, c_int, c_int, ctypes.c_void_p, c_size, c_f32p, c_stream]),
    "st3d_gram_multi_workspace_bytes": (c_size, [ctypes.c_void_p, c_int]),
    "st3d_gram_fwd_multi": (c_int, [ctypes.c_void_p, c_int, ctypes.c_void_p, c_size, c_stream]),
    "st3d_gram_bwd": (c_int, [c_f32p, c_f32p, c_int, c_int, c_int, c_float, c_int, c_f32p, c_stream]),
    "st3d_gram_bwd_gated": (c_int, [c_f32p, c_f32p, c_int, c_int, c_int, c_float, c_int, c_f32p, c_stream]),
    "st3d_guidance_floats": (c_size, [c_int, c_int]),
    "st3d_guidance_partials": (c_size, [c_int, c_int]),
    "st3d_guidance_build": (c_int, [c_f32p, c_int, c_int, c_f32p, c_f32p, c_f32p, c_stream]),
    "st3d_gram_fwd_weighted": (c_int, [c_f32p, c_f32p, c_int, c_int, c_int, ctypes.c_void_p, c_size, c_f32p, c_stream]),
    "st3d_gram_fwd_multi_weighted": (c_int, [ctypes.c_void_p, ctypes.c_void_p, c_int, ctypes.c_void_p, c_size, c_stream]),
    "st3d_gram_bwd_weighted": (c_int, [c_f32p, c_f32p, c_f32p, c_int, c_int, c_int, c_float, c_int, c_int, c_f32p, c_stream]),
    "st3d_reduce_partials": (c_int, []),
    "st3d_sqdiff_sum": (c_int, [c_f32p, c_f32p, c_size, c_size, c_float, c_f32p, c_f32p, c_f32p, c_stream]),
    "st3d_sqdiff_sum_multi": (c_int, [ctypes.c_void_p, c_int, c_f32p, c_f32p, c_int, c_int, c_float, c_float, c_stream]),
    "st3d_axpy_diff": (c_int, [c_f32p, c_f32p, c_size, c_float, c_int, c_f32p, c_stream]),
    "st3d_axpy_diff_gated": (c_int, [c_f32p, c_f32p, c_size, c_float, c_int, c_f32p, c_stream]),
    "st3d_masked_mse": (c_int, [c_f32p, c_f32p, c_f32p, c_int, c_int, c_f32p, c_f32p, c_f32p, c_stream]),
    "st3d_tv_loss": (c_int, [c_f32p, c_f32p, c_int, c_int, c_int, c_int, c_f32p, c_f32p, c_f32p, c_stream]),
    "st3d_range_loss": (c_int, [c_f32p, c_size, c_f32p, c_f32p, c_f32p, c_stream]),
    "st3d_texpyr_numel": (c_size, [c_int, c_int]),
    "st3d_texpyr_synth": (c_int, [c_f32p, c_int, c_int, c_f32p, c_stream]),
    "st3d_texpyr_adjoint": (c_int, [c_f32p, c_int, c_int, c_f32p, c_stream]),
    "st3d_mip_numel": (c_size, [c_int, c_int]),
    "st3d_mip_build": (c_int, [c_f32p, c_int, c_int, c_f32p, c_stream]),
    "st3d_mip_adjoint": (c_int, [c_f32p, c_int, c_int, c_int, c_f32p, c_stream]),
    "st3d_mip_lod": (c_int, [c_i32p, c_f32p, c_f32p, c_f32p, c_i32p, c_f32p, c_i32p, c_int, c_int, c_int, c_int, c_int, c_int,
                             c_int, c_float, c_f32p, c_stream]),
    "st3d_shade_mip_fwd": (c_int, [c_i32p, c_f32p, c_f32p, c_f32p, c_f32p, c_i32p, c_f32p, c_f32p, c_int, c_int, c_int, c_int,
                                   c_int, c_int, c_f32p, c_f32p, c_stream]),
    "st3d_shade_mip_bwd_workspace_bytes": (c_size, [c_int, c_int]),
    "st3d_shade_mip_bwd": (c_int, [c_f32p, c_i32p, c_f32p, c_f32p, c_f32p, c_f32p, c_i32p, c_f32p, c_f32p, c_int, c_int, c_int,
                                   c_int, c_int, c_int, c_f32p, c_f32p, c_f32p, c_f32p, ctypes.c_void_p, c_size, c_stream]),
    "st3d_shade_vc_fwd": (c_int, [c_i32p, c_f32p, c_f32p, c_f32p, c_i32p, c_f32p, c_int, c_int, c_int, c_int, c_f32p, c_f32p,
                                  c_stream]),
    "st3d_shade_vc_bwd": (c_int, [c_f32p, c_i32p, c_f32p, c_f32p, c_f32p, c_i32p, c_f32p, c_int, c_int, c_int, c_int, c_f32p,
                                  c_f32p, c_stream]),
    "st3d_shade_vc_bwd_det_workspace_bytes": (c_size, [c_int]),
    "st3d_shade_vc_bwd_det": (c_int, [c_f32p, c_i32p, c_f32p, c_f32p, c_f32p, c_i32p, c_f32p, c_int, c_int, c_int, c_int, c_f32p,
                                      c_f32p, ctypes.c_void_p, c_size, c_stream]),
    "st3d_atlas_texel_index": (c_int, [c_float, c_float, c_int, ctypes.POINTER(c_int), ctypes.POINTER(c_int)]),
    "st3d_shade_atlas_fwd": (c_int, [c_i32p, c_f32p, c_f32p, c_f32p, c_f32p, c_int, c_int, c_int, c_int, c_f32p, c_f32p,
                                     c_stream]),
    "st3d_shade_atlas_bwd": (c_int, [c_f32p, c_i32p, c_f32p, c_f32p, c_f32p, c_int, c_int, c_int, c_int, c_f32p, c_stream]),
    "st3d_shade_atlas_bwd_det_workspace_bytes": (c_size, [c_int, c_int]),
    "st3d_shade_atlas_bwd_det": (c_int, [c_f32p, c_i32p, c_f32p, c_f32p, c_f32p, c_int, c_int, c_int, c_int, c_f32p,
                                         ctypes.c_void_p, c_size, c_stream]),
    "st3d_adam_step": (c_int, [c_f32p, c_f32p, c_f32p, c_f32p, c_size, c_int, c_float, c_float, c_float, c_float, c_stream]),
    "st3d_diffuse_apply": (c_int, [c_i32p, c_i32p, c_int, c_float, c_f32p, c_f32p, c_stream]),
    "st3d_diffuse_workspace_bytes": (c_size, [c_int]),
    "st3d_diffuse_solve": (c_int, [c_i32p, c_i32p, c_int, c_float, c_f32p, c_f32p, c_float, c_int, ctypes.c_void_p, c_size,
                                   ctypes.c_void_p, c_stream]),
    "st3d_adam_step_uniform": (c_int, [c_f32p, c_f32p, c_f32p, c_f32p, c_size, c_int, c_float, c_float, c_float, c_float, c_f32p,
                                       c_stream]),
    "st3d_cover_mark": (c_int, [c_i32p, c_f32p, c_f32p, c_i32p, c_int, c_int, c_int, ctypes.c_void_p, c_stream]),
    "st3d_cover_workspace_bytes": (c_size, [c_int]),
    "st3d_cover_greedy": (c_int, [ctypes.c_void_p, c_int, c_int, c_int, ctypes.c_void_p, c_i32p, c_i32p, ctypes.c_void_p,
                                  c_stream]),
    "st3d_cover_count": (c_int, [ctypes.c_void_p, c_int, c_int, c_int, c_i32p, c_stream]),
    "st3d_bake_workspace_bytes": (c_size, [c_int]),
    "st3d_bake_surface": (c_int, [c_f32p, c_i32p, c_int, c_int, c_int, c_float, ctypes.c_void_p, c_size, c_i32p, c_f32p, c_stream]),
    "st3d_bake_views": (c_int, [c_f32p, c_i32p, c_int, c_int, c_i32p, c_f32p, c_int, c_f32p, c_f32p, c_f32p, c_i32p, c_f32p, c_int,
                                c_int, c_float, c_int, c_float, c_float, c_float, c_f32p, c_stream]),
    "st3d_bake_resolve": (c_int, [c_f32p, c_f32p, c_int, c_f32p, c_stream]),
    "st3d_fill_workspace_bytes": (c_size, [c_int, c_int]),
    "st3d_fill_pushpull": (c_int, [c_f32p, c_u8p, c_u8p, c_int, c_int, ctypes.c_void_p, c_size, c_f32p, ctypes.c_void_p, c_stream]),
    "st3d_vgg_create": (c_int, [ctypes.POINTER(ctypes.c_void_p)]),
    "st3d_vgg_set_conv": (c_int, [ctypes.c_void_p, c_int, c_f32p, c_f32p, c_stream]),
    "st3d_vgg_destroy": (c_int, [ctypes.c_void_p]),
    "st3d_plan_create": (c_int, [ctypes.POINTER(ctypes.c_void_p), ctypes.c_void_p, c_int, c_int]),
    "st3d_plan_destroy": (c_int, [ctypes.c_void_p]),
    "st3d_plan_bytes": (c_size, [ctypes.c_void_p]),
    "st3d_plan_forward": (c_int, [ctypes.c_void_p, c_f32p, c_int, c_int, c_stream]),
    "st3d_plan_activation": (c_int, [ctypes.c_void_p, c_int, ctypes.POINTER(ctypes.c_void_p), ctypes.POINTER(c_int),
                                     ctypes.POINTER(c_int), ctypes.POINTER(c_int)]),
    "st3d_plan_set_content": (c_int, [ctypes.c_void_p, c_f32p, c_int, c_stream]),
    "st3d_plan_get_content_features": (c_int, [ctypes.c_void_p, c_f32p, c_int, c_stream]),
    "st3d_plan_set_content_features": (c_int, [ctypes.c_void_p, c_f32p, c_int, c_stream]),
    "st3d_plan_set_style": (c_int, [ctypes.c_void_p, c_f32p, c_int, c_int, c_stream]),
    "st3d_plan_set_style_guidance": (c_int, [ctypes.c_void_p, c_f32p, c_int, c_stream]),
    "st3d_plan_loss": (c_int, [ctypes.c_void_p, c_f32p, c_int, c_int, c_float, c_float, c_f32p, c_f32p, c_stream]),
    "st3d_plan_loss_masked": (c_int, [ctypes.c_void_p, c_f32p, c_int, c_int, c_float, c_float, c_f32p, c_f32p, c_u8p, c_stream]),
    "st3d_plan_loss_flat": (c_int, [ctypes.c_void_p, c_f32p, c_int, c_int, c_float, c_float, c_f32p, c_f32p, c_u8p, c_f32p,
                                    c_stream]),
    "st3d_plan_loss_keyed": (c_int, [ctypes.c_void_p, c_f32p, c_int, c_int, c_float, c_float, c_f32p, c_f32p, c_u8p, c_f32p,
                                     ctypes.POINTER(c_float), ctypes.c_uint64, c_stream]),
    "st3d_plan_graph": (c_int, [ctypes.c_void_p, c_int]),
    "st3d_plan_backward": (c_int, [ctypes.c_void_p, c_int, c_int, ctypes.POINTER(ctypes.c_void_p), c_f32p, c_stream]),
    "st3d_comm_unique_id": (c_int, [ctypes.c_char_p]),
    "st3d_comm_init": (c_int, [ctypes.POINTER(ctypes.c_void_p), c_int, c_int, ctypes.c_char_p]),
    "st3d_allreduce_sum_f32": (c_int, [ctypes.c_void_p, c_f32p, c_size, c_stream]),
    "st3d_comm_destroy": (c_int, [ctypes.c_void_p]),
    "st3d_trace_push": (c_int, [ctypes.c_char_p]),
    "st3d_trace_pop": (c_int, []),
    "st3d_trace_enabled": (c_int, []),
    "st3d_plan_split_calls": (c_int, [ctypes.c_void_p, ctypes.POINTER(c_int), ctypes.POINTER(c_int)]),
    "st3d_plan_profile": (c_int, [ctypes.c_void_p, c_int]),
    "st3d_plan_profile_read": (c_int, [ctypes.c_void_p, ctypes.POINTER(c_float), ctypes.POINTER(c_int)]),
    "st3d_plan_profile_launches": (c_int, [ctypes.c_void_p, ctypes.POINTER(c_int), ctypes.POINTER(c_float), c_int,
                                           ctypes.POINTER(c_int)]),
}

_lib = None


class St3dError(RuntimeError):
    pass


def load():
    global _lib
    if _lib is None:
        if not os.path.exists(SO_PATH):
            raise St3dError(f"{SO_PATH} not found: build it with `python 2d-to-3d-style-transfer_amd/build.py` "
                            "(there is no CPU fallback)")
        lib = ctypes.CDLL(SO_PATH)
        for name, (res, args) in SIGNATURES.items():
            fn = getattr(lib, name)
            fn.restype = res
            fn.argtypes = args
        _lib = lib
    return _lib


def check(rc, what=""):
    if rc != 0:
        msg = load().st3d_last_error().decode("utf-8", "replace")
        raise St3dError(f"{what or 'libst3d'} failed (code {rc}): {msg}")


def call(name, *args):
    rc = getattr(load(), name)(*args)
    check(rc, name)


def stream_ptr():
    return ctypes.c_void_p(torch.cuda.current_stream().cuda_stream)


def dptr(t, dtype=None):
    if t is None:
        return None
    if not t.is_cuda:
        raise St3dError("libst3d takes device tensors; got a CPU tensor (no CPU fallback)")
    if not t.is_contiguous():
        raise St3dError("libst3d takes contiguous tensors")
    if t.device.index != torch.cuda.current_device():
        raise St3dError(f"tensor lives on {t.device} but the current device is cuda:{torch.cuda.current_device()}: "
                        "call torch.cuda.set_device(...) (or use `with torch.cuda.device(...)`) first")
    if dtype is not None and t.dtype != dtype:
        raise St3dError(f"expected {dtype}, got {t.dtype}")
    return ctypes.c_void_p(t.data_ptr())
```

2d-to-3d-style-transfer_amd/st3d/ops.py:

```python
import ctypes
import math
import os

import torch

from . import _lib
from ._lib import call, dptr, stream_ptr

F32, I32, U8 = torch.float32, torch.int32, torch.uint8
INV_TAN_HALF_FOV = float(1.0 / math.tan(math.radians(60.0) / 2.0))


def _f32c(t):
    return t.detach().to(F32).contiguous()


_DETERMINISTIC = os.environ.get("ST3D_DETERMINISTIC", "1") not in ("", "0")


def set_deterministic(on=True):
    global _DETERMINISTIC
    _DETERMINISTIC = bool(on)


# ... 1123 lines not shown

def wino_dgrad(gy, act, ud, Cin):
    N, Cout, H, W = gy.shape
    gx = torch.empty((N, Cin, H, W), dtype=F32, device=gy.device)
    call("st3d_wino_dgrad", dptr(gy.contiguous(), F32), dptr(act, F32) if act is not None else None, dptr(ud, F32),
         dptr(gx), N, Cin, Cout, H, W, stream_ptr())
    return gx


def wino_dgrad_unpool(gy_pooled, pool_idx, pooled, ud, Cin):
    N, Cout, Hp, Wp = gy_pooled.shape
    H, W = 2 * Hp, 2 * Wp
    gx = torch.empty((N, Cin, H, W), dtype=F32, device=gy_pooled.device)
    call("st3d_wino_dgrad_unpool", dptr(gy_pooled.contiguous(), F32), dptr(pool_idx, U8), dptr(pooled, F32), dptr(ud, F32),
         dptr(gx), N, Cin, Cout, H, W, stream_ptr())
    return gx


def wino_dgrad_chain(gy, ud, Cin, act=None, pool_idx=None, pooled=None, out_gate=None, add_target=None, add_coef=0.0):
    N, Cout = gy.shape[:2]
    H, W = (2 * gy.shape[2], 2 * gy.shape[3]) if pool_idx is not None else gy.shape[2:]
    gx = torch.empty((N, Cin, H, W), dtype=F32, device=gy.device)
    call("st3d_wino_dgrad_chain", dptr(gy.contiguous(), F32), dptr(act, F32), dptr(pool_idx, U8), dptr(pooled, F32),
         dptr(ud, F32), dptr(out_gate, F32), dptr(add_target, F32), float(add_coef), dptr(gx), N, Cin, Cout, H, W, stream_ptr())
    return gx


def wino43_pack(w):
    w = _f32c(w)
    Cout, Cin = w.shape[:2]
    n = _lib.load().st3d_wino43_packed_floats(Cout, Cin)
    uf = torch.empty((n,), dtype=F32, device=w.device)
    ud = torch.empty((n,), dtype=F32, device=w.device)
    call("st3d_wino43_pack", dptr(w), Cout, Cin, dptr(uf), dptr(ud), stream_ptr())
    return uf, ud


def wino43_fwd(x, uf, bias, Cout, relu=True, pool=False, keep_full=True):
    N, Cin, H, W = x.shape
    y = torch.empty((N, Cout, H, W), dtype=F32, device=x.device) if (keep_full or not pool) else None
    yp = torch.empty((N, Cout, H // 2, W // 2), dtype=F32, device=x.device) if pool else None
    idx = torch.empty((N, Cout, H // 2, W // 2), dtype=U8, device=x.device) if pool else None
    call("st3d_wino43_fwd", dptr(x.contiguous(), F32), dptr(uf, F32), dptr(bias, F32) if bias is not None else None, dptr(y),
         dptr(yp), dptr(idx), N, Cin, Cout, H, W, 1 if relu else 0, stream_ptr())
    return (y, yp, idx) if pool else y


def wino43_dgrad_chain(gy, ud, Cin, pool_idx=None, out_gate=None, add_target=None, add_coef=0.0):
    N, Cout = gy.shape[:2]
    H, W = (2 * gy.shape[2], 2 * gy.shape[3]) if pool_idx is not None else gy.shape[2:]
    gx = torch.empty((N, Cin, H, W), dtype=F32, device=gy.device)
    call("st3d_wino43_dgrad_chain", dptr(gy.contiguous(), F32), dptr(pool_idx, U8), dptr(ud, F32), dptr(out_gate, F32),
         dptr(add_target, F32), float(add_coef), dptr(gx), N, Cin, Cout, H, W, stream_ptr())
    return gx


def wino43_dgrad_chain_tiles(gy, ud, Cin, tile_list, n_active, out, pool_idx=None, out_gate=None, add_target=None, add_coef=0.0,
                             tile_cols=None):
    N, Cout = gy.shape[:2]
    H, W = (2 * gy.shape[2], 2 * gy.shape[3]) if pool_idx is not None else gy.shape[2:]
    assert tuple(out.shape) == (N, Cin, H, W)
    if tile_cols is not None:
        call("st3d_wino43_dgrad_chain_tiles_geo", dptr(gy.contiguous(), F32), dptr(pool_idx, U8), dptr(ud, F32), dptr(out_gate, F32),
             dptr(add_target, F32), float(add_coef), dptr(out, F32), N, Cin, Cout, H, W, int(tile_cols), dptr(tile_list, I32),
             dptr(n_active, I32), stream_ptr())
        return out
    call("st3d_wino43_dgrad_chain_tiles", dptr(gy.contiguous(), F32), dptr(pool_idx, U8), dptr(ud, F32), dptr(out_gate, F32),
         dptr(add_target, F32), float(add_coef), dptr(out, F32), N, Cin, Cout, H, W, dptr(tile_list, I32), dptr(n_active, I32),
         stream_ptr())
    return out


def wino43_fwd_tiles(x, uf, bias, Cout, tile_list, n_active, y=None, yp=None, idx=None, relu=True, tile_cols=None):
    N, Cin, H, W = x.shape
    if tile_cols is not None:
        call("st3d_wino43_fwd_tiles_geo", dptr(x.contiguous(), F32), dptr(uf, F32), dptr(bias, F32), dptr(y, F32), dptr(yp, F32),
             dptr(idx, U8), N, Cin, Cout, H, W, 1 if relu else 0, int(tile_cols), dptr(tile_list, I32), dptr(n_active, I32),
             stream_ptr())
        return
    call("st3d_wino43_fwd_tiles", dptr(x.contiguous(), F32), dptr(uf, F32), dptr(bias, F32), dptr(y, F32), dptr(yp, F32),
         dptr(idx, U8), N, Cin, Cout, H, W, 1 if relu else 0, dptr(tile_list, I32), dptr(n_active, I32), stream_ptr())


def wino43_fwd_strips(x, uf, bias, Cout, strip_list, n_steps, y, relu=True):
    N, Cin, H, W = x.shape
    assert tuple(y.shape) == (N, Cout, H, W)
    call("st3d_wino43_fwd_strips", dptr(x.contiguous(), F32), dptr(uf, F32), dptr(bias, F32), dptr(y, F32), N, Cin, Cout, H, W,
         1 if relu else 0, dptr(strip_list, I32), dptr(n_steps, I32), stream_ptr())
    return y


def kept_build(cover, first=0, nlists=None, tile_cols=None):
    lib = _lib.load()
    N, S, _ = cover.shape
    nlists = need_blocks_lists(S) if nlists is None else nlists
    counts = torch.full((6,), -7, dtype=I32, device=cover.device)
    tcols = [int(c or 0) for c in (tile_cols or [0] * nlists)]
    lists = {k: torch.full((lib.st3d_need_blocks_entries(N, S, k, tcols[k]),), -1, dtype=I32, device=cover.device)
             for k in range(first, nlists)}
    nb = lib.st3d_need_blocks_workspace_bytes(N, S)
    ws = torch.empty((max(nb, 1),), dtype=U8, device=cover.device)
    cols = (ctypes.c_int * max(nlists, 1))(*tcols)
    ptrs = (ctypes.c_void_p * max(nlists, 1))(*[lists[k].data_ptr() if k in lists else None for k in range(nlists)])
    call("st3d_kept_build", dptr(cover, U8), N, S, int(first), nlists, cols, dptr(ws), nb, ptrs, dptr(counts), stream_ptr())
    return {k: (lists[k], counts[k]) for k in lists}


def flat_levels(S):
    return _lib.load().st3d_flat_levels(int(S))


def flat_build(imgs, color, levels=None):
    N, _, S, _ = imgs.shape
    lib = _lib.load()
    levels = flat_levels(S) if levels is None else levels
    nb = lib.st3d_flat_workspace_bytes(N, S)
    ws = torch.empty((max(nb, 16),), dtype=U8, device=imgs.device)
    counts = torch.full((3,), -7, dtype=I32, device=imgs.device)
    lists = [torch.full((lib.st3d_flat_tiles(N, S, k),), -7, dtype=I32, device=imgs.device) for k in range(levels)]
    maps = [torch.full_like(l, -7) for l in lists]
    ptr = lambda seq, k: dptr(seq[k]) if k < len(seq) else None
    call("st3d_flat_build", dptr(imgs, F32), dptr(color, F32), N, S, levels, dptr(ws), nb, ptr(lists, 0), ptr(maps, 0),
         ptr(lists, 1), ptr(maps, 1), ptr(lists, 2), ptr(maps, 2), dptr(counts), stream_ptr())
    return [(lists[k], counts[k], maps[k]) for k in range(levels)]


def flat_fill(tile_map, y=None, yp=None, idx=None):
    t = y if y is not None else yp
    N, C = t.shape[:2]
    H, W = (y.shape[2:] if y is not None else (2 * yp.shape[2], 2 * yp.shape[3]))
    call("st3d_flat_fill", dptr(tile_map, I32), dptr(y, F32), dptr(yp, F32), dptr(idx, U8), N, C, H, W, stream_ptr())


def maxpool2x2(y, want_idx=True):
    N, C, H, W = y.shape
    p = torch.empty((N, C, H // 2, W // 2), dtype=F32, device=y.device)
    idx = torch.empty((N, C, H // 2, W // 2), dtype=U8, device=y.device) if want_idx else None
    call("st3d_maxpool2x2_fwd", dptr(y.contiguous(), F32), dptr(p), dptr(idx), N, C, H, W, stream_ptr())
    return (p, idx) if want_idx else p


GUIDANCE_LEVELS = 5


def guidance_sides(S):
    return [S >> l for l in range(GUIDANCE_LEVELS)]


def _guidance_mask(mask):
    if not torch.is_tensor(mask):
        raise _lib.St3dError("the guidance mask is a tensor (n,1,S,S) or (n,S,S)")
    if mask.dim() == 4 and mask.shape[1] == 1:
        mask = mask[:, 0]
    if mask.dim() != 3 or mask.shape[1] != mask.shape[2] or mask.shape[0] < 1 or mask.shape[1] < 16:
        raise _lib.St3dError(f"the guidance mask is (n,1,S,S) or (n,S,S) with S >= 16; got {tuple(mask.shape)}")
    if not mask.is_cuda:
        raise _lib.St3dError("libst3d takes device tensors; got a CPU mask (no CPU fallback)")
    if mask.dtype != F32:
        raise _lib.St3dError(f"expected {F32}, got {mask.dtype}")
    return mask.detach().contiguous()


def guidance_build(mask):
    m = _guidance_mask(mask)
    n, S = m.shape[0], m.shape[1]
    lib = _lib.load()
    q = torch.empty((lib.st3d_guidance_floats(n, S),), dtype=F32, device=m.device)
    sums = torch.empty((GUIDANCE_LEVELS, n), dtype=F32, device=m.device)
    parts = torch.empty((lib.st3d_guidance_partials(n, S),), dtype=F32, device=m.device)
    call("st3d_guidance_build", dptr(m, F32), n, S, dptr(q), dptr(sums), dptr(parts), stream_ptr())
    planes, off = [], 0
    for H in guidance_sides(S):
        planes.append(q[off:off + n * H * H].view(n, H, H))
        off += n * H * H
    return planes, sums


def _check_q(q, B, HW):
    if q.numel() != B * HW:
        raise _lib.St3dError(f"the weight plane has {q.numel()} values, the features {B} x {HW} pixels")
    return dptr(q.contiguous(), F32)
# ... 312 lines not shown
```

2d-to-3d-style-transfer_amd/st3d/vgg.py:

```python
import ctypes
import math
import os
from collections import OrderedDict

import torch

from . import _lib, ops
from ._lib import call, dptr, stream_ptr

VGG19_CFG = [64, 64, "M", 128, 128, "M", 256, 256, 256, 256, "M", 512, 512, 512, 512, "M", 512, 512, 512, 512, "M"]
DEFAULT_TAPS = {"0": "conv1_1", "5": "conv2_1", "10": "conv3_1", "19": "conv4_1", "21": "conv4_2", "28": "conv5_1"}
STYLE_TAP_MODULES = (0, 5, 10, 19, 28)
CONTENT_TAP_MODULE = 21


def synthetic_state(seed=0, bias_scale=0.05):
    g = torch.Generator().manual_seed(seed)
    state, cin, idx = {}, 3, 0
    for v in VGG19_CFG:
        if v == "M":
            idx += 1
            continue
        state[f"{idx}.weight"] = torch.randn((v, cin, 3, 3), generator=g) * math.sqrt(2.0 / (cin * 9))
        state[f"{idx}.bias"] = torch.randn((v,), generator=g) * bias_scale
# ... 75 lines not shown

    MAX_PLANS = int(os.environ.get("ST3D_MAX_PLANS", "4"))

    def plan(self, B, S):
        key = (int(B), int(S))
        p = self._plans.get(key)
        if p is not None:
            self._plans.move_to_end(key)
            return p
        while len(self._plans) >= max(self.MAX_PLANS, 1):
            self._plans.popitem(last=False)[1].close()
        try:
            p = PerceptualPlan(self, *key)
        except _lib.St3dError:
            if not self._plans:
                raise
            while self._plans:
                self._plans.popitem(last=False)[1].close()
            torch.cuda.empty_cache()
            p = PerceptualPlan(self, *key)
        self._plans[key] = p
        return p

    def __del__(self):
        try:
            for p in list(getattr(self, "_plans", {}).values()):
                p.close()
            if getattr(self, "_h", None):
                _lib.load().st3d_vgg_destroy(self._h)
                self._h = None
        except Exception:
            pass


class PerceptualPlan:

    def __init__(self, vgg, B, S):
        self.vgg, self.B, self.S = vgg, B, S
        h = ctypes.c_void_p()
        call("st3d_plan_create", ctypes.byref(h), vgg._h, B, S)
        self._h = h
        self._content_key = self._style_key = None
        self._content_ref = self._style_ref = None
        self.generation = 0
        self.loss_buf = torch.zeros((3,), dtype=torch.float32, device=vgg.device)
        if os.environ.get("ST3D_GRAPH", "0") not in ("", "0"):
            self.use_graph(True)

    def use_graph(self, on=True):
        call("st3d_plan_graph", self._h, 1 if on else 0)

    def close(self):
        if self._h:
            _lib.load().st3d_plan_destroy(self._h)
            self._h = None

    def bytes(self):
        return _lib.load().st3d_plan_bytes(self._h)

    def forward(self, imgs, upto=28):
        imgs = imgs.detach().to(torch.float32).contiguous()
        call("st3d_plan_forward", self._h, dptr(imgs), imgs.shape[0], int(upto), stream_ptr())
        self._n = imgs.shape[0]
        self.generation += 1

    def backward(self, grads, upto):
        ptrs = (ctypes.c_void_p * 37)()
        keep = []
        for m, g in grads.items():
            g = g.detach().to(torch.float32).contiguous()
            keep.append(g)
            ptrs[int(m)] = g.data_ptr()
        out = torch.empty((self._n, 3, self.S, self.S), dtype=torch.float32, device=self.vgg.device)
        call("st3d_plan_backward", self._h, self._n, int(upto), ptrs, dptr(out), stream_ptr())
        return out

    def activation(self, module_idx, n=None):
        p = ctypes.c_void_p()
        C, H, W = ctypes.c_int(), ctypes.c_int(), ctypes.c_int()
        call("st3d_plan_activation", self._h, int(module_idx), ctypes.byref(p), ctypes.byref(C), ctypes.byref(H),
             ctypes.byref(W))
        n = n or self._n
        return _wrap_device_ptr(p.value, (n, C.value, H.value, W.value), self.vgg.device)

    @staticmethod
    def _key(t):
        return (t.data_ptr(), t._version, tuple(t.shape))

    @staticmethod
    def _same(key, ref, k, t):
        return key is not None and ref is not None and k == key and ref.data_ptr() == t.data_ptr()

    CONTENT_CACHE = 8

    def set_content(self, content, force=False):
        k = self._key(content)
        if not force and self._same(self._content_key, self._content_ref, k, content):
            return
        n = content.shape[0]
        cache = self.__dict__.setdefault("_content_cache", {})
        hit = None if force else cache.get(k)
        if hit is not None:
            call("st3d_plan_set_content_features", self._h, dptr(hit[0]), n, stream_ptr())
        else:
            c = content.detach().to(torch.float32).contiguous()
            call("st3d_plan_set_content", self._h, dptr(c), n, stream_ptr())
            self.generation += 1
            if self._content_key is not None and self.CONTENT_CACHE > 0:
                feats = torch.empty((n, 512, self.S // 8, self.S // 8), dtype=torch.float32, device=self.vgg.device)
                call("st3d_plan_get_content_features", self._h, dptr(feats), n, stream_ptr())
                if len(cache) >= self.CONTENT_CACHE:
                    cache.pop(next(iter(cache)))
                cache[k] = (feats, content)
        self._content_key, self._content_ref = k, content

    def set_style(self, style, n, force=False):
        k = self._key(style) + (n,)
        if force or not self._same(self._style_key, self._style_ref, k, style):
            s = style.detach().to(torch.float32).contiguous()
            sb = s.shape[0]
            if sb > 1 and s.stride(0) == 0:
                sb = 1
            if sb > 1 and bool((s[0:1] == s).all()):
                sb = 1
            s = s[:1].contiguous() if sb == 1 else s
            call("st3d_plan_set_style", self._h, dptr(s), sb, n, stream_ptr())
            self.generation += 1
            self._style_key, self._style_ref = k, style

    @staticmethod
    def _color_key(rgb):
        key = tuple(float(c) for c in rgb)
        if len(key) != 3:
            raise _lib.St3dError(f"flat_color must be 3 floats, got {rgb!r}")
        return key

    def _color(self, rgb):
        key = self._color_key(rgb)
        cache = self.__dict__.setdefault("_colors", {})
        if key not in cache:
            if len(cache) > 64:
                cache.clear()
            cache[key] = torch.tensor(key, dtype=torch.float32, device=self.vgg.device)
        return cache[key]

    def set_style_guidance(self, mask, n=None):
        if mask is None:
            if self.__dict__.get("_guided"):
                call("st3d_plan_set_style_guidance", self._h, None, 0, stream_ptr())
                self._guided = False
            return
        m = mask.detach()
        if m.dim() == 4 and m.shape[1] == 1:
            m = m[:, 0]
        if m.dim() != 3 or tuple(m.shape[1:]) != (self.S, self.S) or (n is not None and m.shape[0] != n):
            raise _lib.St3dError(f"style_mask must be ({n if n is not None else 'n'},1,{self.S},{self.S}) or (n,{self.S},{self.S}), "
                                 f"got {tuple(mask.shape)}")
        if not m.is_cuda:
            raise _lib.St3dError("libst3d takes device tensors; got a CPU style_mask (no CPU fallback)")
        m = m.to(torch.float32).contiguous()
        call("st3d_plan_set_style_guidance", self._h, dptr(m, torch.float32), m.shape[0], stream_ptr())
        self._guided = True

    def loss(self, current, style_weight, content_weight, batch_denom=None, want_grad=True, need_mask=None, flat_color=None,
             style_mask=None, epoch=0):
        cur = current.detach().to(torch.float32).contiguous()
# ... 76 lines not shown
```

include/st3d.h:

```cpp
#ifndef ST3D_H
#define ST3D_H

#include <stddef.h>
#include <stdint.h>

#ifdef __cplusplus
extern "C" {
#endif

#define ST3D_OK 0
#define ST3D_E_INVALID (-1)
#define ST3D_E_HIP (-2)
#define ST3D_E_NOMEM (-3)
#define ST3D_E_STATE (-4)

typedef void *st3d_stream_t;

int st3d_version(void);
const char *st3d_last_error(void);
int st3d_device_info(int device, int *cu_count, size_t *hbm_bytes, char *name, int name_len);


int st3d_project_verts(const float *verts, int V, const float *R, const float *T, int B,
                       float inv_tan_half_fov, float *verts_ndc, st3d_stream_t stream);
// ... 152 lines not shown
                          void *workspace, size_t workspace_bytes, st3d_stream_t stream);
int st3d_box_down_fwd(const float *in, int B, int C, int S, int a, float *out, st3d_stream_t stream);
int st3d_box_down_bwd(const float *grad_out, int B, int C, int S, int a, float *grad_in, st3d_stream_t stream);

int st3d_apply_background(const float *img, const float *mask, const float *bg, int bg_batch,
                          int B, int S, float *out, st3d_stream_t stream);


size_t st3d_conv3x3_packed_floats(int Cout, int Cin);
int st3d_conv3x3_pack(const float *w, int Cout, int Cin, float *w_fwd, float *w_dgrad,
                      st3d_stream_t stream);
int st3d_conv3x3_fwd(const float *x, const float *w_fwd_packed, const float *bias, float *y,
                     int N, int Cin, int Cout, int H, int W, int relu, st3d_stream_t stream);
size_t st3d_conv1_skip_tiles(int N, int H, int W);
int st3d_conv1_skip_build(const uint8_t *cover, int N, int H, int W, uint8_t *skip, st3d_stream_t stream);
int st3d_conv3x3_fwd_skip(const float *x, const float *w_fwd_packed, const float *bias, float *y, int N, int Cin, int Cout,
                          int H, int W, int relu, const uint8_t *tile_skip, st3d_stream_t stream);
int st3d_conv3x3_dgrad(const float *gy, const float *act, const float *w_dgrad_packed, float *gx,
                       int N, int Cin, int Cout, int H, int W, st3d_stream_t stream);
int st3d_conv1_bwd_supported(int H, int W);
size_t st3d_conv1_bwd_workspace_bytes(int N, int H, int W);
int st3d_conv1_bwd(const float *gy, const float *act, const float *D, float coef, const float *w_dgrad_packed,
                   void *workspace, size_t workspace_bytes, float *gx, int N, int H, int W, st3d_stream_t stream);
int st3d_conv1_bwd_masked(const float *gy, const float *act, const float *D, float coef, const float *w_dgrad_packed,
                          void *workspace, size_t workspace_bytes, float *gx, int N, int H, int W, const uint8_t *seg,
                          const uint8_t *mask, st3d_stream_t stream);
int st3d_conv1_bwd_weighted(const float *gy, const float *act, const float *D, float coef, const float *w_dgrad_packed,
                            void *workspace, size_t workspace_bytes, float *gx, int N, int H, int W, const float *w0,
                            const uint8_t *seg, const uint8_t *mask, st3d_stream_t stream);
int st3d_conv3x3_dgrad_unpool(const float *gy_pooled, const uint8_t *pool_idx, const float *pooled,
                              const float *w_dgrad_packed, float *gx, int N, int Cin, int Cout,
                              int H, int W, st3d_stream_t stream);
int st3d_wino_supported(int Cin, int Cout, int H, int W);
size_t st3d_wino_packed_floats(int Cout, int Cin);
int st3d_wino_pack(const float *w, int Cout, int Cin, float *u_fwd, float *u_dgrad, st3d_stream_t stream);
int st3d_wino_fwd(const float *x, const float *u_fwd, const float *bias, float *y, float *y_pooled,
                  uint8_t *pool_idx, int N, int Cin, int Cout, int H, int W, int relu, st3d_stream_t stream);
int st3d_wino_dgrad(const float *gy, const float *act, const float *u_dgrad, float *gx, int N, int Cin,
                    int Cout, int H, int W, st3d_stream_t stream);
int st3d_wino_dgrad_unpool(const float *gy_pooled, const uint8_t *pool_idx, const float *pooled,
                           const float *u_dgrad, float *gx, int N, int Cin, int Cout, int H, int W,
                           st3d_stream_t stream);
int st3d_wino_dgrad_chain(const float *gy, const float *act, const uint8_t *pool_idx, const float *pooled,
                          const float *u_dgrad, const float *out_gate, const float *add_target, float add_coef,
                          float *gx, int N, int Cin, int Cout, int H, int W, st3d_stream_t stream);
int st3d_wino43_supported(int Cin, int Cout, int H, int W);
size_t st3d_wino43_packed_floats(int Cout, int Cin);
int st3d_wino43_pack(const float *w, int Cout, int Cin, float *u_fwd, float *u_dgrad, st3d_stream_t stream);
int st3d_wino43_fwd(const float *x, const float *u_fwd, const float *bias, float *y, float *y_pooled, uint8_t *pool_idx,
                    int N, int Cin, int Cout, int H, int W, int relu, st3d_stream_t stream);
int st3d_wino43_dgrad_chain(const float *gy, const uint8_t *pool_idx, const float *u_dgrad, const float *out_gate,
                            const float *add_target, float add_coef, float *gx, int N, int Cin, int Cout, int H, int W,
                            st3d_stream_t stream);
int st3d_wino43_tile_geometry(int H, int W, int *rows, int *cols);
int st3d_wino43_dgrad_chain_tiles(const float *gy, const uint8_t *pool_idx, const float *u_dgrad, const float *out_gate,
                                  const float *add_target, float add_coef, float *gx, int N, int Cin, int Cout, int H, int W,
                                  const int *tile_list, const int *n_active, st3d_stream_t stream);
int st3d_need_levels(int S);
size_t st3d_need_workspace_bytes(int N, int S);
int st3d_need_build(const uint8_t *mask, int N, int S, int levels, uint8_t *seg, void *workspace, size_t workspace_bytes,
                    int *list1, int *list2, int *counts, st3d_stream_t stream);
#define ST3D_NEED_MAX_LISTS 6
int st3d_need_blocks_lists(int S);
size_t st3d_need_blocks_tiles(int N, int S, int k);
size_t st3d_need_blocks_entries(int N, int S, int k, int tile_cols);
size_t st3d_need_blocks_workspace_bytes(int N, int S);
size_t st3d_need_blocks_gram_runs(int N, int S);
int st3d_need_blocks_build(const uint8_t *mask, int N, int S, int nlists, const int *tile_cols, uint8_t *seg, void *workspace,
                           size_t workspace_bytes, int *const *lists, int *counts, int *gram_list, int *gram_count,
                           st3d_stream_t stream);
int st3d_gram_bwd_segs_supported(int C, int HW);
int st3d_gram_bwd_gated_segs(const float *D, const float *feat, const float *q, int B, int C, int HW, float coef, int accumulate,
                             const int *seg_list, const int *seg_count, float *gfeat, st3d_stream_t stream);
int st3d_wino43_dgrad_chain_tiles_geo(const float *gy, const uint8_t *pool_idx, const float *u_dgrad, const float *out_gate,
                                      const float *add_target, float add_coef, float *gx, int N, int Cin, int Cout, int H, int W,
                                      int tile_cols, const int *tile_list, const int *n_active, st3d_stream_t stream);
int st3d_wino43_fwd_tiles_geo(const float *x, const float *u_fwd, const float *bias, float *y, float *y_pooled, uint8_t *pool_idx,
                              int N, int Cin, int Cout, int H, int W, int relu, int tile_cols, const int *tile_list,
                              const int *n_active, st3d_stream_t stream);
int st3d_wino43_fwd_strips(const float *x, const float *u_fwd, const float *bias, float *y, int N, int Cin, int Cout, int H,
                           int W, int relu, const int *strip_list, const int *n_steps, st3d_stream_t stream);
int st3d_kept_build(const uint8_t *cover, int N, int S, int first, int nlists, const int *tile_cols, void *workspace,
                    size_t workspace_bytes, int *const *lists, int *counts, st3d_stream_t stream);
int st3d_wino43_fwd_tiles(const float *x, const float *u_fwd, const float *bias, float *y, float *y_pooled, uint8_t *pool_idx,
                          int N, int Cin, int Cout, int H, int W, int relu, const int *tile_list, const int *n_active,
                          st3d_stream_t stream);
int st3d_flat_levels(int S);
int st3d_flat_tiles(int N, int S, int launch );
size_t st3d_flat_workspace_bytes(int N, int S);
int st3d_flat_build(const float *imgs, const float *color, int N, int S, int levels, void *workspace, size_t workspace_bytes,
                    int *list1, int *map1, int *list2, int *map2, int *list3, int *map3, int *counts, st3d_stream_t stream);
int st3d_flat_fill(const int *tile_map, float *y, float *y_pooled, uint8_t *pool_idx, int N, int C, int H, int W,
                   st3d_stream_t stream);
int st3d_flat_build_cover(const uint8_t *cover, int N, int S, int levels, void *workspace, size_t workspace_bytes, int *list1,
                          int *map1, int *list2, int *map2, int *list3, int *map3, int *counts, st3d_stream_t stream);
int st3d_flat_check_cover(const float *imgs, const float *color, const uint8_t *cover, int N, int S, void *workspace,
                          size_t workspace_bytes, int *bad, st3d_stream_t stream);
int st3d_maxpool2x2_fwd(const float *y, float *p, uint8_t *idx, int N, int C, int H, int W,
                        st3d_stream_t stream);


size_t st3d_gram_workspace_bytes(int B, int C, int HW);
int st3d_gram_fwd(const float *feat, int B, int C, int HW, void *workspace, size_t workspace_bytes,
                  float *gram, st3d_stream_t stream);
typedef struct st3d_gram_item {
    const float *feat;
    float *gram;
    int B, C, HW;
} st3d_gram_item;
size_t st3d_gram_multi_workspace_bytes(const st3d_gram_item *items, int count);
int st3d_gram_fwd_multi(const st3d_gram_item *items, int count, void *workspace, size_t workspace_bytes,
                        st3d_stream_t stream);
int st3d_gram_bwd(const float *D, const float *feat, int B, int C, int HW, float coef,
                  int accumulate, float *gfeat, st3d_stream_t stream);
int st3d_gram_bwd_gated(const float *D, const float *feat, int B, int C, int HW, float coef,
                        int accumulate, float *gfeat, st3d_stream_t stream);
size_t st3d_guidance_floats(int n, int S);
size_t st3d_guidance_partials(int n, int S);
int st3d_guidance_build(const float *mask, int n, int S, float *q_out, float *sums_out, float *partials,
                        st3d_stream_t stream);
int st3d_gram_fwd_weighted(const float *feat, const float *q, int B, int C, int HW, void *workspace,
                           size_t workspace_bytes, float *gram, st3d_stream_t stream);
int st3d_gram_fwd_multi_weighted(const st3d_gram_item *items, const float *const *q, int count, void *workspace,
                                 size_t workspace_bytes, st3d_stream_t stream);
int st3d_gram_bwd_weighted(const float *D, const float *feat, const float *q, int B, int C, int HW, float coef,
                           int accumulate, int gated, float *gfeat, st3d_stream_t stream);
int st3d_reduce_partials(void);
int st3d_sqdiff_sum(const float *a, const float *b, size_t n, size_t nb, float scale, float *D,
                    float *partials, float *loss_out, st3d_stream_t stream);
typedef struct st3d_sqdiff_item {
    const float *a; const float *b; float *D;
    size_t n, nb;
    float scale;
    int slot;
} st3d_sqdiff_item;
int st3d_sqdiff_sum_multi(const st3d_sqdiff_item *items, int count, float *partials, float *loss_out3,
                          int zero_first, int combine, float style_weight, float content_weight,
                          st3d_stream_t stream);
int st3d_axpy_diff(const float *a, const float *b, size_t n, float coef, int accumulate, float *g,
                   st3d_stream_t stream);
int st3d_axpy_diff_gated(const float *a, const float *b, size_t n, float coef, int accumulate, float *g,
                         st3d_stream_t stream);
int st3d_masked_mse(const float *rendered, const float *target, const float *mask, int B, int S,
                    float *grad_rendered, float *partials, float *loss_out, st3d_stream_t stream);
int st3d_tv_loss(const float *images, const float *masks, int B, int C, int H, int W, float *partials,
                 float *loss_and_mask_sum, float *grad_images, st3d_stream_t stream);
int st3d_range_loss(const float *values, size_t n, float *partials, float *loss_out, float *grad, st3d_stream_t stream);

size_t st3d_mesh_reg_scratch_floats(int V, int P);
int st3d_mesh_reg(const float *verts, const float *target_verts, int V, const int32_t *edges, int E,
                  const int32_t *nbr_off, const int32_t *nbr_idx, const int32_t *pairs, int P,
                  const int32_t *pair_off, const int32_t *pair_ref,
                  const float *weights, float *scratch, float *partials, float *loss_out,
                  float *grad_verts, st3d_stream_t stream);

size_t st3d_mesh_reg_ex_scratch_floats(int V, int E, int F, int P);
int st3d_mesh_reg_ex(const float *verts, const float *target_verts, int V, const int32_t *edges, int E,
                     const int32_t *nbr_off, const int32_t *nbr_idx, const int32_t *pairs, int P,
                     const int32_t *pair_off, const int32_t *pair_ref, const int32_t *faces, int F,
                     const int32_t *nbr_edge, const int32_t *edge_off, const int32_t *edge_ref,
                     const int32_t *inc_off, const int32_t *inc_ref, int laplacian_method, float edge_target_length,
                     const float *weights, float *scratch, float *partials, float *loss_out,
                     float *grad_verts, st3d_stream_t stream);

int st3d_knn1_geometry(int P1, int P2, int *tile, int *segments);
size_t st3d_knn1_workspace_bytes(int P1, int P2);
// ... 11 lines not shown
int st3d_chamfer_sum(const float *dist, int P, double scale, float *loss, st3d_stream_t stream);
int st3d_chamfer_bwd(const float *x, const float *y, int P1, int P2, const int32_t *nn, const int32_t *order,
                     const int32_t *sorted, double c_self, double c_other, float *grad_x, st3d_stream_t stream);

int st3d_nnfm_geometry(int N, int M, int C, int *tile_q, int *tile_s, int *segments);
size_t st3d_nnfm_workspace_bytes(int B, int N, int M, int C);
int st3d_nnfm_normalise(const float *x, int B, int C, int M, float *xhat, float *norm, st3d_stream_t stream);
int st3d_nnfm_search(const float *feat_hat, const float *feat_norm, const float *style_hat, const float *weights, int B, int Bs,
                     int C, int N, int M, void *workspace, size_t workspace_bytes, int32_t *idx, float *dist,
                     st3d_stream_t stream);
int st3d_nnfm_sum(const float *dist, const float *weights, int B, int N, double inv_denom, float *loss, double *wsum,
                  st3d_stream_t stream);
int st3d_nnfm_bwd(const float *feat, const float *style_hat, const int32_t *idx, const float *dist,
                  const float *weights, const double *wsum, const float *grad_out, int B, int Bs, int C, int N, int M,
                  double inv_denom, float *grad_feat, st3d_stream_t stream);

int st3d_swd_project(const float *x, const float *a, int B, int Q, int R, int N, float *out, st3d_stream_t stream);
int st3d_swd_geometry(int N, int *block, int *passes);
size_t st3d_swd_workspace_bytes(int B, int K, int N);
int st3d_swd_sort(const float *proj, const float *weights, int B, int K, int N, void *workspace, size_t workspace_bytes,
                  float *sorted, int32_t *perm, int32_t *count, st3d_stream_t stream);
int st3d_swd_loss(const float *sorted, const int32_t *count, const float *tsorted, int B, int Bs, int K, int N, int M,
                  double inv_denom, void *workspace, size_t workspace_bytes, float *loss, st3d_stream_t stream);
int st3d_swd_bwd(const float *sorted, const int32_t *perm, const int32_t *count, const float *tsorted, const float *grad_out,
                 int B, int Bs, int K, int N, int M, double inv_denom, float *gproj, st3d_stream_t stream);

size_t st3d_texpyr_numel(int T, int L);
int st3d_texpyr_synth(const float *params, int T, int L, float *texture, st3d_stream_t stream);
int st3d_texpyr_adjoint(const float *grad_texture, int T, int L, float *grad_params, st3d_stream_t stream);

size_t st3d_mip_numel(int T, int L);
int st3d_mip_build(const float *texture, int T, int L, float *pyramid, st3d_stream_t stream);
int st3d_mip_adjoint(const float *grad_pyramid, int T, int L, int accumulate, float *grad_texture, st3d_stream_t stream);
int st3d_mip_lod(const int32_t *pix_to_face, const float *bary, const float *zbuf, const float *verts_ndc,
                 const int32_t *faces, const float *verts_uvs, const int32_t *faces_uvs, int B, int S, int T, int L, int V,
                 int F, int VT, float bias, float *lod, st3d_stream_t stream);
int st3d_shade_mip_fwd(const int32_t *pix_to_face, const float *bary, const float *zbuf, const float *dists,
                       const float *verts_uvs, const int32_t *faces_uvs, const float *pyramid, const float *lod, int B, int S,
                       int T, int L, int F, int VT, float *rgb, float *mask, st3d_stream_t stream);
size_t st3d_shade_mip_bwd_workspace_bytes(int T, int L);
int st3d_shade_mip_bwd(const float *grad_rgb, const int32_t *pix_to_face, const float *bary, const float *zbuf,
                       const float *dists, const float *verts_uvs, const int32_t *faces_uvs, const float *pyramid,
                       const float *lod, int B, int S, int T, int L, int F, int VT, float *grad_pyramid, float *grad_texture,
                       float *grad_uv, float *grad_bary, void *workspace, size_t workspace_bytes, st3d_stream_t stream);

int st3d_shade_vc_fwd(const int32_t *pix_to_face, const float *bary, const float *zbuf, const float *dists,
                      const int32_t *faces, const float *verts_colors, int B, int S, int F, int V, float *rgb, float *mask,
                      st3d_stream_t stream);
int st3d_shade_vc_bwd(const float *grad_rgb, const int32_t *pix_to_face, const float *bary, const float *zbuf,
                      const float *dists, const int32_t *faces, const float *verts_colors, int B, int S, int F, int V,
                      float *grad_colors, float *grad_bary, st3d_stream_t stream);
size_t st3d_shade_vc_bwd_det_workspace_bytes(int V);
int st3d_shade_vc_bwd_det(const float *grad_rgb, const int32_t *pix_to_face, const float *bary, const float *zbuf,
                          const float *dists, const int32_t *faces, const float *verts_colors, int B, int S, int F, int V,
                          float *grad_colors, float *grad_bary, void *workspace, size_t workspace_bytes,
                          st3d_stream_t stream);

int st3d_atlas_texel_index(float b0, float b1, int R, int *wy, int *wx);
int st3d_shade_atlas_fwd(const int32_t *pix_to_face, const float *bary, const float *zbuf, const float *dists,
                         const float *atlas, int B, int S, int F, int R, float *rgb, float *mask, st3d_stream_t stream);
int st3d_shade_atlas_bwd(const float *grad_rgb, const int32_t *pix_to_face, const float *bary, const float *zbuf,
                         const float *dists, int B, int S, int F, int R, float *grad_atlas, st3d_stream_t stream);
size_t st3d_shade_atlas_bwd_det_workspace_bytes(int F, int R);
int st3d_shade_atlas_bwd_det(const float *grad_rgb, const int32_t *pix_to_face, const float *bary, const float *zbuf,
                             const float *dists, int B, int S, int F, int R, float *grad_atlas, void *workspace,
                             size_t workspace_bytes, st3d_stream_t stream);

int st3d_adam_step(float *param, const float *grad, float *exp_avg, float *exp_avg_sq, size_t n,
                   int step, float lr, float beta1, float beta2, float eps, st3d_stream_t stream);

typedef struct st3d_vgg st3d_vgg;
typedef struct st3d_plan st3d_plan;

int st3d_vgg_create(st3d_vgg **out);
int st3d_vgg_set_conv(st3d_vgg *vgg, int module_idx, const float *w, const float *b,
                      st3d_stream_t stream);
int st3d_vgg_destroy(st3d_vgg *vgg);

int st3d_plan_create(st3d_plan **out, st3d_vgg *vgg, int B, int S);
int st3d_plan_destroy(st3d_plan *plan);
size_t st3d_plan_bytes(const st3d_plan *plan);
int st3d_plan_forward(st3d_plan *plan, const float *imgs, int n, int upto_module, st3d_stream_t stream);
int st3d_plan_activation(st3d_plan *plan, int module_idx, float **ptr, int *C, int *H, int *W);
int st3d_plan_set_content(st3d_plan *plan, const float *content, int n, st3d_stream_t stream);
int st3d_plan_get_content_features(st3d_plan *plan, float *out, int n, st3d_stream_t stream);
int st3d_plan_set_content_features(st3d_plan *plan, const float *features, int n, st3d_stream_t stream);
int st3d_plan_set_style(st3d_plan *plan, const float *style, int style_batch, int n, st3d_stream_t stream);
int st3d_plan_set_style_guidance(st3d_plan *plan, const float *mask, int n, st3d_stream_t stream);
int st3d_plan_loss(st3d_plan *plan, const float *current, int n, int batch_denom, float style_weight,
                   float content_weight, float *loss_out, float *grad_current, st3d_stream_t stream);
int st3d_plan_loss_masked(st3d_plan *plan, const float *current, int n, int batch_denom, float style_weight,
                          float content_weight, float *loss_out, float *grad_current, const uint8_t *need_mask,
                          st3d_stream_t stream);
int st3d_plan_loss_flat(st3d_plan *plan, const float *current, int n, int batch_denom, float style_weight,
                        float content_weight, float *loss_out, float *grad_current, const uint8_t *need_mask,
                        const float *flat_color, st3d_stream_t stream);
int st3d_plan_loss_keyed(st3d_plan *plan, const float *current, int n, int batch_denom, float style_weight,
                         float content_weight, float *loss_out, float *grad_current, const uint8_t *cover,
                         const float *flat_color, const float *flat_rgb, uint64_t epoch, st3d_stream_t stream);
int st3d_plan_split_calls(const st3d_plan *plan, int *forward_calls, int *backward_calls);
int st3d_plan_graph(st3d_plan *plan, int enable);
int st3d_plan_backward(st3d_plan *plan, int n, int upto_module, const float *const *grad_modules, float *grad_image,
                       st3d_stream_t stream);
#define ST3D_PROFILE_FAMILIES 16
int st3d_plan_profile(st3d_plan *plan, int enable);
int st3d_plan_profile_read(st3d_plan *plan, float *ms_out ,
                           int *launches_out );
int st3d_plan_profile_launches(st3d_plan *plan, int *tags_out , float *ms_out ,
                               int capacity, int *count_out);

int st3d_diffuse_apply(const int *nbr_off, const int *nbr_idx, int V, float lambda, const float *x, float *y,
                       st3d_stream_t stream);
size_t st3d_diffuse_workspace_bytes(int V);
int st3d_diffuse_solve(const int *nbr_off, const int *nbr_idx, int V, float lambda, const float *b, float *x, float tol,
                       int max_iter, void *workspace, size_t workspace_bytes, void *info, st3d_stream_t stream);
int st3d_adam_step_uniform(float *param, const float *grad, float *exp_avg, float *exp_avg_sq, size_t n, int step, float lr,
                           float beta1, float beta2, float eps, float *partials, st3d_stream_t stream);

int st3d_cover_mark(const int32_t *pix_to_face, const float *bary, const float *verts_uvs, const int32_t *faces_uvs, int B,
                    int S, int T, void *masks , st3d_stream_t stream);
size_t st3d_cover_workspace_bytes(int C);
int st3d_cover_greedy(const void *masks , int C, int W, int n, void *covered , int32_t *picks ,
                      int32_t *gains , void *workspace, st3d_stream_t stream);
int st3d_cover_count(const void *masks , int C, int W, int T, int32_t *counts , st3d_stream_t stream);

#define ST3D_BAKE_MEAN 0
#define ST3D_BAKE_BEST 1
size_t st3d_bake_workspace_bytes(int T);
int st3d_bake_surface(const float *verts_uvs, const int32_t *faces_uvs, int VT, int F, int T, float pad, void *workspace,
                      size_t workspace_bytes, int32_t *t2f, float *tbary, st3d_stream_t stream);
int st3d_bake_views(const float *verts, const int32_t *faces, int V, int F, const int32_t *t2f, const float *tbary, int Tt,
                    const float *R, const float *T, const float *images, const int32_t *pix_to_face, const float *zbuf, int B,
                    int S, float inv_tan_half_fov, int mode, float power, float min_cos, float depth_tol, float *acc,
                    st3d_stream_t stream);
int st3d_bake_resolve(const float *acc, const float *fallback, int Tt, float *out, st3d_stream_t stream);

size_t st3d_fill_workspace_bytes(int H, int W);
int st3d_fill_pushpull(const float *tex, const uint8_t *valid, const uint8_t *domain, int H, int W, void *workspace,
                       size_t workspace_bytes, float *out, int64_t *count, st3d_stream_t stream);

#define ST3D_COMM_ID_BYTES 128
typedef struct st3d_comm st3d_comm;
int st3d_comm_unique_id(unsigned char id_out[ST3D_COMM_ID_BYTES]);
int st3d_comm_init(st3d_comm **out, int rank, int world, const unsigned char unique_id[ST3D_COMM_ID_BYTES]);
int st3d_allreduce_sum_f32(st3d_comm *comm, float *buf , size_t n, st3d_stream_t stream);
int st3d_comm_destroy(st3d_comm *comm);

int st3d_trace_push(const char *name);
int st3d_trace_pop(void);
int st3d_trace_enabled(void);

#ifdef __cplusplus
}
#endif
#endif
```

Measured before the change: 140.2 iter/s (one iter = 8 views of 512x512: render + VGG-19 fwd/bwd + Gram/content loss + Adam).

## Run pooled VGG convs over kept strip lists with fused max-pool epilogue

Lets the Winograd 4x3 strip-list forward path also take the fused 2x2 max-pool epilogue, so pooling convolution layers (conv1_2, conv2_2, conv3_4) compute only kept strips and write pooled outputs plus argmax directly. It extends the kept-list builder with a seventh list for conv3_4 and adds per-level pooled enable logic based on a two-rounds occupancy heuristic. The aim is to skip background work and the separate pool pass at these layers. In exchange it adds list-build and bookkeeping complexity, and untouched pooled entries depend on fill correctness.

Result: no change. 141.3 iter/s (one iter = 8 views of 512x512: render + VGG-19 fwd/bwd + Gram/content loss + Adam) (median of 6 runs) (+0.8%).

```diff
diff --git a/2d-to-3d-style-transfer_amd/csrc/need.hip b/2d-to-3d-style-transfer_amd/csrc/need.hip
--- a/2d-to-3d-style-transfer_amd/csrc/need.hip
+++ b/2d-to-3d-style-transfer_amd/csrc/need.hip
@@ -94,18 +94,20 @@
 }
 
 constexpr int kLists = ST3D_NEED_MAX_LISTS;
-constexpr int kListShift[kLists] = {0, 1, 1, 2, 2, 2};
-constexpr int kListUnpools[kLists] = {1, 0, 1, 0, 0, 0};
+constexpr int kKept = ST3D_KEPT_MAX_LISTS;
+static_assert(kKept == kLists + 1, "the kept lists: the need lists' launches and conv3_4");
+constexpr int kListShift[kKept] = {0, 1, 1, 2, 2, 2, 2};
+constexpr int kListUnpools[kKept] = {1, 0, 1, 0, 0, 0, 0};
 
 struct BlockLevels {
     int nlists;
     int first;
-    int bw[kLists];
-    int trows[kLists], tcols[kLists];
-    int unpools[kLists];
+    int bw[kKept];
+    int trows[kKept], tcols[kKept];
+    int unpools[kKept];
     int N;
-    int total[kLists + 1];
-    int *list[kLists];
+    int total[kKept + 1];
+    int *list[kKept];
     int gram_runs;
     int *gram_list, *gram_count;
 };
@@ -421,6 +423,17 @@
     return (size_t)N * bw * bw / 16;
 }
 
+extern "C" int st3d_kept_lists(int S) {
+    const int n = st3d_need_blocks_lists(S);
+    return n == kLists ? kKept : n;
+}
+
+extern "C" size_t st3d_kept_entries(int N, int S, int k, int tile_cols) {
+    if (N <= 0 || k < 0 || k >= st3d_kept_lists(S)) return 0;
+    const size_t bw = (size_t)(S >> kListShift[k]) / 4;
+    return (size_t)N * bw * bw / 16 * (tile_cols == 16 ? 4 : 1);
+}
+
 extern "C" size_t st3d_need_blocks_entries(int N, int S, int k, int tile_cols) {
     return st3d_need_blocks_tiles(N, S, k) * (tile_cols == 16 ? 4 : 1);
 }
@@ -459,7 +472,7 @@
         L.trows[k] = cols == 32 ? 2 : 1;
         L.tcols[k] = cols / 4;
         L.unpools[k] = kListUnpools[k];
-        L.total[k] = (int)st3d_need_blocks_tiles(N, S, k);
+        L.total[k] = (int)st3d_kept_entries(N, S, k, 0);
         L.list[k] = k < first ? nullptr : lists[k];
     }
     return ST3D_OK;
@@ -497,7 +510,7 @@
 extern "C" int st3d_kept_build(const uint8_t *cover, int N, int S, int first, int nlists, const int *tile_cols, void *workspace,
                                size_t workspace_bytes, int *const *lists, int *counts, st3d_stream_t stream) {
     ST3D_CHECK_ARG(cover && N > 0);
-    ST3D_CHECK_ARG(first >= 0 && first < nlists && nlists <= st3d_need_blocks_lists(S));
+    ST3D_CHECK_ARG(first >= 0 && first < nlists && nlists <= st3d_kept_lists(S));
     ST3D_CHECK_ARG(((uintptr_t)cover & 15) == 0);
     ST3D_CHECK_ARG((long)N * S * S < (1L << 31));
     ST3D_CHECK_ARG(lists && counts && workspace && workspace_bytes >= st3d_need_blocks_workspace_bytes(N, S));
diff --git a/2d-to-3d-style-transfer_amd/csrc/plan.hip b/2d-to-3d-style-transfer_amd/csrc/plan.hip
--- a/2d-to-3d-style-transfer_amd/csrc/plan.hip
+++ b/2d-to-3d-style-transfer_amd/csrc/plan.hip
@@ -176,7 +176,7 @@
         uint8_t *need_seg = nullptr;
         int *need_list[ST3D_NEED_MAX_LISTS] = {}, *need_cnt = nullptr;
         int *need_gram_list = nullptr, *need_gram_cnt = nullptr;
-        int *kept_list[ST3D_NEED_MAX_LISTS] = {}, *kept_cnt = nullptr;
+        int *kept_list[ST3D_KEPT_MAX_LISTS] = {}, *kept_cnt = nullptr;
         int *flat_list[3] = {}, *flat_map[3] = {}, *flat_cnt = nullptr;
     };
     struct ListSet {
@@ -259,6 +259,7 @@
     const st3d_plan::Lists &lists;
     const uint8_t *c1_skip;
     const bool *kept_on;
+    const bool *pooled_on;
 };
 
 bool split_ok(const st3d_plan *p, int dir, int n, bool keyed) {
@@ -291,7 +292,7 @@
     }
     if (want_kept) {
         Scope sc(p, F_ELEM, s);
-        ST3D_TRY(st3d_kept_build(cover, images, p->S, p->d.keep_first, kKeepFirst + p->d.keep_levels, p->d.keep_cols, p->keep_ws,
+        ST3D_TRY(st3d_kept_build(cover, images, p->S, p->d.build_first, p->d.build_end, p->d.build_cols, p->keep_ws,
                                  p->keep_ws_bytes, L.kept_list, L.kept_cnt, s));
     }
     return ST3D_OK;
@@ -310,6 +311,8 @@
     const st3d_vgg *v = p->vgg;
     const int m = kConvIdx[cs], k = cs - 1, Cin = kConvCin[cs], Cout = kConvCout[cs], H = p->H[m], W = p->W[m];
     Scope sc(p, F_CONV43_FWD_FLAT, s, m);
+    if (cols == 16 && yp)
+        return st3d_wino43_fwd_strips_pool(x, v->u6f[cs], v->bias[cs], y, yp, yi, n, Cin, Cout, H, W, 1, L.kept_list[k], L.kept_cnt + k, s);
     if (cols == 16) return st3d_wino43_fwd_strips(x, v->u6f[cs], v->bias[cs], y, n, Cin, Cout, H, W, 1, L.kept_list[k], L.kept_cnt + k, s);
     return st3d_wino43_fwd_tiles_geo(x, v->u6f[cs], v->bias[cs], y, yp, yi, n, Cin, Cout, H, W, 1, cols, L.kept_list[k], L.kept_cnt + k, s);
 }
@@ -347,7 +350,12 @@
             float *yp = pps >= 0 ? act(pool_m) : nullptr;
             uint8_t *yi = pps >= 0 ? p->at(p->pidx[pps], pool_m, i0) : nullptr;
             const bool listed = cs >= 1 && (cs <= flat || (cs > kKeepFirst && cs <= kKeepFirst + keep));
-            const int kept_cols = !(listed && !fill && keep > 0 && on(cs - 1)) ? 0 : cs <= flat ? p->d.shallow_cols[cs - 1] : p->d.keep_cols[cs - 1];
+            int kept_cols = !(listed && cs <= ST3D_NEED_MAX_LISTS && !fill && keep > 0 && on(cs - 1)) ? 0
+                            : cs <= flat                                                      ? p->d.shallow_cols[cs - 1]
+                                                                                              : p->d.keep_cols[cs - 1];
+            const int pl = pooled_level(cs);
+            if (pl >= 0 && p->d.pooled_cols[pl] && listed && !fill && keep > 0)
+                kept_cols = (pps >= 0 && (!fl.pooled_on || fl.pooled_on[pl])) ? 16 : 0;
             if (kept_cols) {
                 ST3D_TRY(kept_launch(p, cs, x, yfull, yp, yi, n, kept_cols, L, s));
             } else if (cs >= 1 && cs <= flat) {
@@ -388,6 +396,7 @@
     int keep = 0;
     if (key && flat == p->d.flat_levels)
         while (keep < p->d.keep_levels && kConvIdx[kKeepFirst + 1 + keep] <= upto) ++keep;
+    if (keep == kKeepMax && p->d.pooled_cols[kPooledLevels - 1] && kConvIdx[kKeepFirst + 1 + kKeepMax] + 2 <= upto) ++keep;
     const bool fill = !(key && flat > 0 && p->clean.matches(key->epoch, n, flat, key->rgb, v->sets, keep));
     p->clean.clear();
     if (flat > 0 && !key) {
@@ -420,11 +429,11 @@
         ls->have_grp_fwd = true;
         ST3D_TRY(run_split(p, 0, s, [&](int g, hipStream_t gs) {
             const FwdLists fl{ls->grp[g], ls->c1_skip ? ls->c1_skip + st3d_conv1_skip_tiles(1, p->S, p->S) * (size_t)g * h : nullptr,
-                              p->d.grp_kept_on};
+                              p->d.grp_kept_on, p->d.grp_pooled_on};
             return forward_chain(p, imgs + (size_t)g * h * 3 * p->S * p->S, g * h, h, upto, keep_full, gs, flat, keep, fill, fl);
         }));
     } else {
-        ST3D_TRY(forward_chain(p, imgs, 0, n, upto, keep_full, s, flat, keep, fill, FwdLists{ls->whole, ls->c1_skip, nullptr}));
+        ST3D_TRY(forward_chain(p, imgs, 0, n, upto, keep_full, s, flat, keep, fill, FwdLists{ls->whole, ls->c1_skip, nullptr, nullptr}));
     }
     p->last_n = n;
     return ST3D_OK;
@@ -616,9 +625,9 @@
             }
         }
         if (kept) {
-            alloc(&L.kept_cnt, (size_t)ST3D_NEED_MAX_LISTS);
-            for (int k = d.keep_first; k < kKeepFirst + d.keep_levels; ++k)
-                alloc(&L.kept_list[k], st3d_need_blocks_entries(images, S, k, d.keep_cols[k]));
+            alloc(&L.kept_cnt, (size_t)std::max(d.build_end, ST3D_NEED_MAX_LISTS));
+            for (int k = d.build_first; k < d.build_end; ++k)
+                alloc(&L.kept_list[k], st3d_kept_entries(images, S, k, d.build_cols[k]));
         }
     };
     if (d.split_mode && rc == ST3D_OK) {
@@ -672,6 +681,15 @@
 extern "C" int st3d_plan_activation(st3d_plan *p, int module_idx, float **ptr, int *C, int *H, int *W) {
     ST3D_CHECK_ARG(p && ptr && module_idx >= 0 && module_idx < kModules);
     *ptr = p->act[module_idx];
+    if (C) *C = p->C[module_idx];
+    if (H) *H = p->H[module_idx];
+    if (W) *W = p->W[module_idx];
+    return ST3D_OK;
+}
+
+extern "C" int st3d_plan_pool_argmax(st3d_plan *p, int module_idx, uint8_t **ptr, int *C, int *H, int *W) {
+    ST3D_CHECK_ARG(p && ptr && module_idx >= 0 && module_idx < kModules && pool_slot(module_idx) >= 0);
+    *ptr = p->pidx[pool_slot(module_idx)];
     if (C) *C = p->C[module_idx];
     if (H) *H = p->H[module_idx];
     if (W) *W = p->W[module_idx];
diff --git a/2d-to-3d-style-transfer_amd/csrc/planlists.h b/2d-to-3d-style-transfer_amd/csrc/planlists.h
--- a/2d-to-3d-style-transfer_amd/csrc/planlists.h
+++ b/2d-to-3d-style-transfer_amd/csrc/planlists.h
@@ -38,6 +38,13 @@
 #define ST3D_SPLIT_BATCH_DEFAULT 1
 enum { SPLIT_FWD = 1, SPLIT_BWD = 2 };
 constexpr int kKeepFirst = 3, kKeepMax = 3;
+constexpr int kPooledLevels = 3;
+constexpr int kPooledSlot[kPooledLevels] = {1, 3, 7}, kPooledList[kPooledLevels] = {0, 2, 6};
+inline int pooled_level(int cs) {
+    for (int i = 0; i < kPooledLevels; ++i)
+        if (kPooledSlot[i] == cs) return i;
+    return -1;
+}
 
 struct PlanFacts {
     int B = 0, S = 0, cus = 0;
@@ -64,6 +71,10 @@
     bool grp_kept_on[ST3D_NEED_MAX_LISTS] = {};
     int grp_need_levels = 0;
     bool grp_need_gram = false;
+    int pooled_cols[kPooledLevels] = {};
+    bool grp_pooled_on[kPooledLevels] = {};
+    int build_first = kKeepFirst, build_end = kKeepFirst;
+    int build_cols[ST3D_KEPT_MAX_LISTS] = {};
 };
 
 inline int next_cols(const char *&cur, int dflt, bool last_repeats) {
@@ -155,6 +166,31 @@
     for (int cs = 3; cs <= ST3D_NEED_MAX_LISTS && cs + 1 <= d.grp_need_levels; ++cs)
         if (!need_force && !two_rounds(hb, f.H[cs], kConvCin[cs])) d.grp_need_levels = cs;
     d.grp_need_gram = d.need_gram && (need_force || gram_rounds(hb));
+
+    static const int kDefaultPooled[kPooledLevels] = {16, 16, 16};
+    const bool pooled_force = flag("ST3D_POOLED_FORCE", false);
+    const char *pc = env("ST3D_KEEP_POOLED");
+    for (int i = 0; i < kPooledLevels; ++i) {
+        const int cs = kPooledSlot[i], k = kPooledList[i], R = f.H[cs], cols = next_cols(pc, kDefaultPooled[i], false);
+        const int geo = k < ST3D_NEED_MAX_LISTS ? k : ST3D_NEED_MAX_LISTS - 1;
+        const bool below = k < kKeepFirst ? d.keep_levels >= 1 : (d.keep_levels == kKeepMax && f.blocks_lists == ST3D_NEED_MAX_LISTS);
+        if (cols != 16 || !below || route[cs].fwd != WINO43 || !pools(cs) || f.geo_rows[geo] == 0) continue;
+        if (!pooled_force && !two_rounds(B, R, kConvCout[cs])) continue;
+        d.pooled_cols[i] = 16;
+        d.grp_pooled_on[i] = pooled_force || two_rounds(hb, R, kConvCout[cs]);
+    }
+    d.build_first = d.keep_first;
+    d.build_end = kKeepFirst + d.keep_levels;
+    for (int k = 0; k < ST3D_NEED_MAX_LISTS; ++k) d.build_cols[k] = d.keep_cols[k];
+    for (int i = 0; i < kPooledLevels; ++i) {
+        if (!d.pooled_cols[i]) continue;
+        const int k = kPooledList[i];
+        d.build_cols[k] = 16;
+        d.build_first = std::min(d.build_first, k);
+        d.build_end = std::max(d.build_end, k + 1);
+    }
+    for (int k = d.build_first; k < 3; ++k)
+        if (!d.build_cols[k]) d.build_cols[k] = d.shallow_cols[k] ? d.shallow_cols[k] : 16;
     return d;
 }
 
diff --git a/2d-to-3d-style-transfer_amd/csrc/wino43.hip b/2d-to-3d-style-transfer_amd/csrc/wino43.hip
--- a/2d-to-3d-style-transfer_amd/csrc/wino43.hip
+++ b/2d-to-3d-style-transfer_amd/csrc/wino43.hip
@@ -69,7 +69,8 @@
 template <int MODE, int EPI, int GATE, int BH, int TC, bool LIST, bool STRIPS>
 __device__ __forceinline__ void wino43_body(const Wino43Args &a, float *smem) {
     using G = Geo43<TC>;
-    static_assert(!STRIPS || (LIST && EPI == 0 && G::TR == 4), "strips come from a list and leave through the plain epilogue");
+    static_assert(!STRIPS || (LIST && G::TR == 4 && (EPI == 0 || (MODE == 0 && GATE == 0))),
+                  "strips come from a list; the fused pool behind them belongs to the plain forward");
     constexpr int SROWS = STRIPS ? 4 : G::ROWS;
     const int tid = threadIdx.x;
     const int lane = tid & 63, wave = __builtin_amdgcn_readfirstlane(tid >> 6);
@@ -551,7 +552,7 @@
 }
 
 template <int MODE, int TC>
-int launch_wino43_tc(Wino43Args a, hipStream_t s, bool strip_fwd = false) {
+int launch_wino43_tc(Wino43Args a, hipStream_t s, bool strip_fwd = false, bool strip_pool = false) {
     using G = Geo43<TC>;
     constexpr bool kStrips = TC == 4;
     a.tiles_x = a.W / G::COLS;
@@ -583,13 +584,21 @@
     if constexpr (kStrips) {
         if (!a.tile_list || !a.n_active) { st3d::set_error("wino43: 16-pixel tile columns come with a strip list and its count"); return ST3D_E_INVALID; }
         if (((uintptr_t)a.tile_list & 15) != 0) { st3d::set_error("wino43: a strip list is 16-byte aligned"); return ST3D_E_INVALID; }
-        if (a.yp) { st3d::set_error("wino43: strip lists leave through the plain epilogue, not the fused pool"); return ST3D_E_INVALID; }
+        if (a.yp && !(strip_fwd && strip_pool && MODE == 0 && !a.gate)) { st3d::set_error("wino43: strip lists leave through the plain epilogue, not the fused pool"); return ST3D_E_INVALID; }
         if ((a.bias || a.relu) && !(strip_fwd && MODE == 0 && !a.gate)) { st3d::set_error("wino43: strip lists are for the input-gradient chain"); return ST3D_E_INVALID; }
         if (a.gate && a.addt) {
             if (MODE != 0) { st3d::set_error("wino43: the content-target term rides on ungated input (MODE 0) only"); return ST3D_E_INVALID; }
             return go(wino43_kernel<0, 0, 2, TC, true, true>);
         }
         if (a.gate) return go(wino43_kernel<MODE, 0, 1, TC, true, true>);
+        if constexpr (MODE == 0) {
+            if (a.yp) {
+                auto kernel = wino43_kernel<0, 1, 0, TC, true, true>;
+                static const hipError_t attr = hipFuncSetAttribute(reinterpret_cast<const void *>(kernel), hipFuncAttributeMaxDynamicSharedMemorySize, (int)kSmem);
+                if (attr != hipSuccess) { st3d::set_error("wino43: hipFuncSetAttribute(MaxDynamicSharedMemorySize): %s", hipGetErrorString(attr)); return ST3D_E_HIP; }
+                return go(kernel);
+            }
+        }
         return go(wino43_kernel<MODE, 0, 0, TC, true, true>);
     } else {
     if (a.tile_list) {
@@ -617,7 +626,7 @@
 }
 
 template <int MODE>
-int launch_wino43(Wino43Args a, hipStream_t s, int cols = 0, bool strip_fwd = false) {
+int launch_wino43(Wino43Args a, hipStream_t s, int cols = 0, bool strip_fwd = false, bool strip_pool = false) {
     const int native = tc43(a.H, a.W);
     if (cols != 0 && !((cols == 64 && native == 16) || (cols == 32 && a.H > 0 && a.W > 0 && (a.H % 8) == 0 && (a.W % 32) == 0) ||
                        (cols == 16 && native != 0))) {
@@ -625,7 +634,7 @@
         return ST3D_E_INVALID;
     }
     const int tc = cols ? cols / 4 : native;
-    if (tc == 4) return launch_wino43_tc<MODE, 4>(a, s, strip_fwd);
+    if (tc == 4) return launch_wino43_tc<MODE, 4>(a, s, strip_fwd, strip_pool);
     return tc == 16 ? launch_wino43_tc<MODE, 16>(a, s) : launch_wino43_tc<MODE, 8>(a, s);
 }
 
@@ -692,6 +701,18 @@
     a.tile_list = strip_list;
     a.n_active = n_steps;
     return launch_wino43<0>(a, st3d::as_stream(stream), 16, true);
+}
+
+extern "C" int st3d_wino43_fwd_strips_pool(const float *x, const float *u_fwd, const float *bias, float *y, float *y_pooled,
+                                           uint8_t *pool_idx, int N, int Cin, int Cout, int H, int W, int relu,
+                                           const int *strip_list, const int *n_steps, st3d_stream_t stream) {
+    ST3D_CHECK_ARG(x && u_fwd && y_pooled && strip_list && n_steps);
+    ST3D_CHECK_ARG(N > 0 && shape_ok43(Cin, Cout, H, W));
+    ST3D_CHECK_ARG(((uintptr_t)u_fwd & 15) == 0);
+    Wino43Args a{x, nullptr, u_fwd, bias, y, y_pooled, pool_idx, N, Cin, Cout, H, W, relu, 0, 0, 0, nullptr, nullptr, 0.f};
+    a.tile_list = strip_list;
+    a.n_active = n_steps;
+    return launch_wino43<0>(a, st3d::as_stream(stream), 16, true, true);
 }
 
 extern "C" int st3d_wino43_dgrad_chain(const float *gy, const uint8_t *pool_idx, const float *u_dgrad, const float *out_gate,
diff --git a/2d-to-3d-style-transfer_amd/st3d/_lib.py b/2d-to-3d-style-transfer_amd/st3d/_lib.py
--- a/2d-to-3d-style-transfer_amd/st3d/_lib.py
+++ b/2d-to-3d-style-transfer_amd/st3d/_lib.py
@@ -202,6 +202,10 @@
                                        c_stream]),
     "st3d_kept_build": (c_int, [c_u8p, c_int, c_int, c_int, c_int, ctypes.POINTER(c_int), ctypes.c_void_p, c_size,
                                 ctypes.POINTER(ctypes.c_void_p), c_i32p, c_stream]),
+    "st3d_kept_lists": (c_int, [c_int]),
+    "st3d_kept_entries": (c_size, [c_int, c_int, c_int, c_int]),
+    "st3d_wino43_fwd_strips_pool": (c_int, [c_f32p, c_f32p, c_f32p, c_f32p, c_f32p, c_u8p, c_int, c_int, c_int, c_int, c_int, c_int,
+                                            c_i32p, c_i32p, c_stream]),
     "st3d_maxpool2x2_fwd": (c_int, [c_f32p, c_f32p, c_u8p, c_int, c_int, c_int, c_int, c_stream]),
     "st3d_gram_workspace_bytes": (c_size, [c_int, c_int, c_int]),
     "st3d_gram_fwd": (c_int, [c_f32p, c_int, c_int, c_int, ctypes.c_void_p, c_size, c_f32p, c_stream]),
@@ -278,6 +282,8 @@
     "st3d_plan_forward": (c_int, [ctypes.c_void_p, c_f32p, c_int, c_int, c_stream]),
     "st3d_plan_activation": (c_int, [ctypes.c_void_p, c_int, ctypes.POINTER(ctypes.c_void_p), ctypes.POINTER(c_int),
                                      ctypes.POINTER(c_int), ctypes.POINTER(c_int)]),
+    "st3d_plan_pool_argmax": (c_int, [ctypes.c_void_p, c_int, ctypes.POINTER(ctypes.c_void_p), ctypes.POINTER(c_int),
+                                      ctypes.POINTER(c_int), ctypes.POINTER(c_int)]),
     "st3d_plan_set_content": (c_int, [ctypes.c_void_p, c_f32p, c_int, c_stream]),
     "st3d_plan_get_content_features": (c_int, [ctypes.c_void_p, c_f32p, c_int, c_stream]),
     "st3d_plan_set_content_features": (c_int, [ctypes.c_void_p, c_f32p, c_int, c_stream]),
diff --git a/2d-to-3d-style-transfer_amd/st3d/ops.py b/2d-to-3d-style-transfer_amd/st3d/ops.py
--- a/2d-to-3d-style-transfer_amd/st3d/ops.py
+++ b/2d-to-3d-style-transfer_amd/st3d/ops.py
@@ -1229,21 +1229,31 @@
          dptr(idx, U8), N, Cin, Cout, H, W, 1 if relu else 0, dptr(tile_list, I32), dptr(n_active, I32), stream_ptr())
 
 
-def wino43_fwd_strips(x, uf, bias, Cout, strip_list, n_steps, y, relu=True):
+def wino43_fwd_strips(x, uf, bias, Cout, strip_list, n_steps, y, relu=True, yp=None, idx=None):
     N, Cin, H, W = x.shape
-    assert tuple(y.shape) == (N, Cout, H, W)
+    assert y is None or tuple(y.shape) == (N, Cout, H, W)
+    if yp is not None:
+        assert tuple(yp.shape) == (N, Cout, H // 2, W // 2) and (idx is None or tuple(idx.shape) == tuple(yp.shape))
+        call("st3d_wino43_fwd_strips_pool", dptr(x.contiguous(), F32), dptr(uf, F32), dptr(bias, F32), dptr(y, F32), dptr(yp, F32),
+             dptr(idx, U8), N, Cin, Cout, H, W, 1 if relu else 0, dptr(strip_list, I32), dptr(n_steps, I32), stream_ptr())
+        return yp
+    assert y is not None and idx is None
     call("st3d_wino43_fwd_strips", dptr(x.contiguous(), F32), dptr(uf, F32), dptr(bias, F32), dptr(y, F32), N, Cin, Cout, H, W,
          1 if relu else 0, dptr(strip_list, I32), dptr(n_steps, I32), stream_ptr())
     return y
+
+
+def kept_lists(S):
+    return _lib.load().st3d_kept_lists(int(S))
 
 
 def kept_build(cover, first=0, nlists=None, tile_cols=None):
     lib = _lib.load()
     N, S, _ = cover.shape
     nlists = need_blocks_lists(S) if nlists is None else nlists
-    counts = torch.full((6,), -7, dtype=I32, device=cover.device)
+    counts = torch.full((7,), -7, dtype=I32, device=cover.device)
     tcols = [int(c or 0) for c in (tile_cols or [0] * nlists)]
-    lists = {k: torch.full((lib.st3d_need_blocks_entries(N, S, k, tcols[k]),), -1, dtype=I32, device=cover.device)
+    lists = {k: torch.full((lib.st3d_kept_entries(N, S, k, tcols[k]),), -1, dtype=I32, device=cover.device)
              for k in range(first, nlists)}
     nb = lib.st3d_need_blocks_workspace_bytes(N, S)
     ws = torch.empty((max(nb, 1),), dtype=U8, device=cover.device)
diff --git a/2d-to-3d-style-transfer_amd/st3d/vgg.py b/2d-to-3d-style-transfer_amd/st3d/vgg.py
--- a/2d-to-3d-style-transfer_amd/st3d/vgg.py
+++ b/2d-to-3d-style-transfer_amd/st3d/vgg.py
@@ -181,6 +181,15 @@
              ctypes.byref(W))
         n = n or self._n
         return _wrap_device_ptr(p.value, (n, C.value, H.value, W.value), self.vgg.device)
+
+    def pool_argmax(self, module_idx, n=None):
+        p = ctypes.c_void_p()
+        C, H, W = ctypes.c_int(), ctypes.c_int(), ctypes.c_int()
+        call("st3d_plan_pool_argmax", self._h, int(module_idx), ctypes.byref(p), ctypes.byref(C), ctypes.byref(H), ctypes.byref(W))
+        n = n or self._n
+        count = n * C.value * H.value * W.value
+        assert count % 4 == 0
+        return _wrap_device_ptr(p.value, (count // 4,), self.vgg.device).view(torch.uint8).view(n, C.value, H.value, W.value)
 
     @staticmethod
     def _key(t):
diff --git a/include/st3d.h b/include/st3d.h
--- a/include/st3d.h
+++ b/include/st3d.h
@@ -258,6 +258,12 @@
                            int W, int relu, const int *strip_list, const int *n_steps, st3d_stream_t stream);
 int st3d_kept_build(const uint8_t *cover, int N, int S, int first, int nlists, const int *tile_cols, void *workspace,
                     size_t workspace_bytes, int *const *lists, int *counts, st3d_stream_t stream);
+#define ST3D_KEPT_MAX_LISTS 7
+int st3d_kept_lists(int S);
+size_t st3d_kept_entries(int N, int S, int k, int tile_cols);
+int st3d_wino43_fwd_strips_pool(const float *x, const float *u_fwd, const float *bias, float *y, float *y_pooled,
+                                uint8_t *pool_idx, int N, int Cin, int Cout, int H, int W, int relu, const int *strip_list,
+                                const int *n_steps, st3d_stream_t stream);
 int st3d_wino43_fwd_tiles(const float *x, const float *u_fwd, const float *bias, float *y, float *y_pooled, uint8_t *pool_idx,
                           int N, int Cin, int Cout, int H, int W, int relu, const int *tile_list, const int *n_active,
                           st3d_stream_t stream);
@@ -435,6 +441,7 @@
 size_t st3d_plan_bytes(const st3d_plan *plan);
 int st3d_plan_forward(st3d_plan *plan, const float *imgs, int n, int upto_module, st3d_stream_t stream);
 int st3d_plan_activation(st3d_plan *plan, int module_idx, float **ptr, int *C, int *H, int *W);
+int st3d_plan_pool_argmax(st3d_plan *plan, int module_idx, uint8_t **ptr, int *C, int *H, int *W);
 int st3d_plan_set_content(st3d_plan *plan, const float *content, int n, st3d_stream_t stream);
 int st3d_plan_get_content_features(st3d_plan *plan, float *out, int n, st3d_stream_t stream);
 int st3d_plan_set_content_features(st3d_plan *plan, const float *features, int n, st3d_stream_t stream);
```
